# youdie006/CLAP2Diffusion

Measured on AMD Instinct MI355X. Metric: 512x512 images/sec @ 50 DDIM steps, batch=8, 1/2/4/8 MI355X, higher is better.
Workload: dtype fp16; 1 GPU; c3: batch=8/GPU, 50 DDIM steps, 512x512, CFG 7.5, log-mel+HTSAT+projectors+CLIP+UNet+VAE, all-gather of images; global_batch=8, ddim_steps=50, resolution=512, parallelism=dp1

## Files before the change

clap2diffusion_amd/_lib.py:

```python
from __future__ import annotations

import ctypes
import os
from ctypes import c_float, c_int, c_size_t, c_void_p
from pathlib import Path

import torch

LIB_PATH = Path(os.environ.get("C2D_LIB") or Path(__file__).resolve().parent / "libc2d_hip.so")

C2D_PRO_NONE, C2D_PRO_GN, C2D_PRO_LN, C2D_PRO_SILU, C2D_PRO_LNFOLD = 0, 1, 2, 3, 4
C2D_PAD_SAME, C2D_PAD_AFTER = 0, 1
C2D_ACT = {None: 0, "none": 0, "geglu": 1, "gelu": 2, "relu": 3, "silu": 4, "quick_gelu": 5}
ERRORS = {-1: "C2D_E_ARG", -2: "C2D_E_SHAPE", -3: "C2D_E_ALIGN", -4: "C2D_E_HIP"}

EXPORTS = [
    "c2d_conv2d_igemm", "c2d_conv2d_igemm_workspace_size", "c2d_conv2d_igemm_plan", "c2d_set_plan_override", "c2d_get_plan_override", "c2d_groupnorm_workspace_size", "c2d_groupnorm_stats", "c2d_groupnorm_apply", "c2d_groupnorm_run_workspace_size", "c2d_groupnorm", "c2d_groupnorm_pad_workspace_size", "c2d_groupnorm_pad", "c2d_conv2d_gn_rows", "c2d_groupnorm_moments", "c2d_layernorm_stats",
    "c2d_layernorm", "c2d_attention_fwd", "c2d_attention_fwd_bias", "c2d_attention_fwd_mask", "c2d_window_attention", "c2d_htsat_mel_patches",
    "c2d_patch_merge_gather", "c2d_row_mean", "c2d_l2_normalize", "c2d_softmax_rows", "c2d_clap_log_mel", "c2d_attention_small", "c2d_pack_weights", "c2d_timestep_embedding",
    "c2d_cfg_ddim_step", "c2d_latent_to_nhwc", "c2d_upsample_nearest2x", "c2d_add", "c2d_last_hip_error", "c2d_version",
    "c2d_image_to_nhwc", "c2d_vae_posterior_noise",
    "c2d_cfg_ddim_step_masked", "c2d_mask_to_latent", "c2d_composite_u8",
    "c2d_inpaint_prepare",
]


class ConvDesc(ctypes.Structure):
    _fields_ = [
        ("src0", c_void_p), ("src1", c_void_p), ("c0", c_int), ("c1", c_int),
        ("n", c_int), ("h", c_int), ("w", c_int), ("oh", c_int), ("ow", c_int),
        ("ksize", c_int), ("stride", c_int), ("up", c_int),
        ("weight", c_void_p), ("cout", c_int), ("kpad", c_int),
        ("pro", c_int), ("pro_silu", c_int), ("pro_a", c_void_p), ("pro_b", c_void_p),
        ("gamma", c_void_p), ("beta", c_void_p), ("bias", c_void_p), ("act", c_int),
        ("temb", c_void_p), ("temb_ld", c_int), ("resid", c_void_p), ("resid_ld", c_int),
        ("out", c_void_p), ("out_ld", c_int), ("ws", c_void_p), ("ws_bytes", c_size_t),
        ("src_pad", c_int), ("pro_eps", c_float),
        ("gn_mom", c_void_p), ("gn_groups", c_int),
        ("pad_mode", c_int),
    ]


_lib = None


def lib() -> ctypes.CDLL:
    global _lib
    if _lib is not None:
        return _lib
    if not LIB_PATH.exists():
        raise RuntimeError(
            f"{LIB_PATH} is missing: build it with `python -m clap2diffusion_amd.build` "
            "(the HIP library is the only compute path; there is no fallback)")
    L = ctypes.CDLL(str(LIB_PATH))
    vp, i, f, sz = c_void_p, c_int, c_float, c_size_t
    sig = {
        "c2d_conv2d_igemm": ([ctypes.POINTER(ConvDesc), vp], i),
        "c2d_conv2d_igemm_workspace_size": ([ctypes.POINTER(ConvDesc)], sz),
        "c2d_conv2d_igemm_plan": ([ctypes.POINTER(ConvDesc), ctypes.POINTER(c_int), ctypes.POINTER(c_int)], i),
        "c2d_set_plan_override": ([i, i], i),
        "c2d_get_plan_override": ([ctypes.POINTER(ctypes.c_int), ctypes.POINTER(ctypes.c_int)], i),
        "c2d_groupnorm_workspace_size": ([i, i, i], sz),
        "c2d_groupnorm_stats": ([vp, vp, i, i, i, i, i, f, vp, vp, vp, vp, vp, vp], i),
        "c2d_groupnorm_apply": ([vp, vp, i, i, i, i, vp, vp, i, vp, vp], i),
        "c2d_groupnorm_run_workspace_size": ([i, i, i, i], sz),
        "c2d_groupnorm": ([vp, vp, i, i, i, i, i, f, vp, vp, i, vp, vp, sz, vp], i),
        "c2d_groupnorm_pad_workspace_size": ([i, i, i, i], sz),
        "c2d_groupnorm_pad": ([vp, vp, i, i, i, i, i, i, f, vp, vp, i, vp, vp, sz, vp], i),
        "c2d_conv2d_gn_rows": ([ctypes.POINTER(ConvDesc)], i),
        "c2d_groupnorm_moments": ([vp, i, i, i, i, f, vp, vp, i, vp, i, i, vp, vp], i),
        "c2d_layernorm_stats": ([vp, i, i, i, f, vp, vp], i),
        "c2d_layernorm": ([vp, i, i, i, f, vp, vp, vp, i, vp], i),
        "c2d_attention_fwd": ([vp, i, vp, i, vp, i, vp, i, i, i, i, i, i, f, i, vp], i),
        "c2d_attention_fwd_bias": ([vp, i, vp, i, vp, i, vp, i, i, i, i, i, i, f, i, vp, i, i, vp], i),
        "c2d_attention_fwd_mask": ([vp, i, vp, i, vp, i, vp, i, i, i, i, i, i, f, i, vp, i, i, i, vp], i),
        "c2d_window_attention": ([vp, i, vp, i, i, i, vp, vp, i, vp, i, vp], i),
        "c2d_htsat_mel_patches": ([vp, i, i, vp, vp, vp, vp], i),
        "c2d_patch_merge_gather": ([vp, i, i, i, i, vp, vp], i),
        "c2d_row_mean": ([vp, i, i, i, i, vp, vp], i),
        "c2d_l2_normalize": ([vp, i, i, vp], i),
        "c2d_softmax_rows": ([vp, i, i, i, vp, i, vp], i),
        "c2d_clap_log_mel": ([vp, vp, vp, i, i, i, i, vp, vp, vp, i, vp, vp], i),
        "c2d_attention_small": ([vp, i, vp, i, vp, i, vp, i, i, i, i, i, f, i, vp], i),
        "c2d_pack_weights": ([vp, i, i, i, i, i, vp, vp], i),
        "c2d_timestep_embedding": ([vp, vp, i, i, vp, vp], i),
        "c2d_cfg_ddim_step": ([vp, vp, i, i, i, f, vp, vp, i, vp], i),
        "c2d_latent_to_nhwc": ([vp, i, i, i, i, i, vp, vp], i),
        "c2d_upsample_nearest2x": ([vp, i, i, i, i, vp, vp], i),
        "c2d_image_to_nhwc": ([vp, i, i, vp, vp], i),
        "c2d_vae_posterior_noise": ([vp, i, vp, vp, vp, vp, i, i, f, vp, vp], i),
        "c2d_cfg_ddim_step_masked": ([vp, vp, vp, vp, vp, i, i, i, f, vp, vp, i, vp], i),
        "c2d_mask_to_latent": ([vp, i, i, i, vp, vp], i),
        "c2d_composite_u8": ([vp, vp, vp, sz, vp, vp], i),
        "c2d_inpaint_prepare": ([vp, i, vp, vp, vp, vp, vp, i, i, i, i, f, vp, vp, vp, vp], i),
        "c2d_add": ([vp, vp, vp, sz, vp], i),
        "c2d_last_hip_error": ([], i),
        "c2d_version": ([], ctypes.c_char_p),
    }
    for name, (args, res) in sig.items():
        fn = getattr(L, name)
        fn.argtypes = args
        fn.restype = res
    _lib = L
    return L


def check(rc: int, what: str) -> None:
    if rc != 0:
        extra = ""
        if rc == -4:
            extra = f" (hipError {lib().c2d_last_hip_error()})"
        raise RuntimeError(f"{what} failed: {ERRORS.get(rc, rc)}{extra}")


def stream_ptr() -> int:
    return torch.cuda.current_stream().cuda_stream


def ptr(t) -> int | None:
    if t is None:
        return None
    return t.data_ptr()


def is_available() -> bool:
    return LIB_PATH.exists()


os.environ.setdefault("HSA_ENABLE_IPC_MODE_LEGACY", "0")
```

clap2diffusion_amd/csrc/norm.hip:

```cpp
#include "common.h"
#include <stdlib.h>

namespace c2d {

__device__ __forceinline__ float gn_read(const f16* s0, const f16* s1, int c0, int c1, size_t pix, int c) {
    return (float)((c < c0) ? s0[pix * c0 + c] : s1[pix * c1 + (c - c0)]);
}

template <int CPT, bool GP = false>
__global__ void __launch_bounds__(256) gn_partial_kernel(const f16* __restrict__ s0, const f16* __restrict__ s1,
                                                         int c0, int c1, int hw, int cpg, int rows_per_block,
                                                         float* __restrict__ ws) {
    extern __shared__ __attribute__((aligned(16))) float red[];
    const int cin = c0 + c1, nch = cin >> 3;
    const int n = blockIdx.y;
    const int t = threadIdx.x;
    const int R = (CPT == 1) ? (256 / nch) : 1;
    const int ch_base = (CPT == 1) ? (t % nch) : t;
    const int r0 = (CPT == 1) ? (t / nch) : 0;
    const bool active = (CPT == 1) ? (t < R * nch) : true;
    const int p_begin = blockIdx.x * rows_per_block;
    const int p_end = min(hw, p_begin + rows_per_block);
    const size_t img = (size_t)n * hw;

    float sum[CPT][8], sq[CPT][8], shift[CPT][8];
#pragma unroll
    for (int q = 0; q < CPT; ++q)
#pragma unroll
        for (int i = 0; i < 8; ++i) { sum[q][i] = 0.f; sq[q][i] = 0.f; shift[q][i] = 0.f; }

    if (active) {
        auto ld8 = [&](int pix, int q) {
            const size_t gp = img + pix;
            const int c = (ch_base + q * 256) * 8;
            const f16* ptr = (c < c0) ? (s0 + gp * c0 + c) : (s1 + gp * c1 + (c - c0));
            return *reinterpret_cast<const f16x8*>(ptr);
        };
        auto acc8 = [&](const f16x8& v, int q) {
#pragma unroll
            for (int i = 0; i < 8; ++i) {
                float d = (float)v[i] - shift[q][i];
                sum[q][i] += d;
                sq[q][i] += d * d;
            }
        };
        constexpr int UN = CPT == 1 ? 8 : 4;
        int pix = p_begin + r0;
        bool first = true;
        for (; pix + (UN - 1) * R < p_end; pix += UN * R) {
            f16x8 v[UN][CPT];
#pragma unroll
            for (int u = 0; u < UN; ++u)
#pragma unroll
                for (int q = 0; q < CPT; ++q)
                    if (q == 0 || ch_base + q * 256 < nch) v[u][q] = ld8(pix + u * R, q);
            if (first) {
#pragma unroll
                for (int q = 0; q < CPT; ++q) {
                    const int ch = ch_base + q * 256;
                    if (ch >= nch) continue;
#pragma unroll
                    for (int i = 0; i < 8; ++i) shift[q][i] = gn_read(s0, s1, c0, c1, img, ((ch * 8 + i) / cpg) * cpg);
                }
                first = false;
            }
            asm volatile("" ::: "memory");
#pragma unroll
            for (int u = 0; u < UN; ++u)
#pragma unroll
                for (int q = 0; q < CPT; ++q)
                    if (q == 0 || ch_base + q * 256 < nch) acc8(v[u][q], q);
        }
        if (first) {
#pragma unroll
            for (int q = 0; q < CPT; ++q) {
                const int ch = ch_base + q * 256;
                if (ch >= nch) continue;
#pragma unroll
                for (int i = 0; i < 8; ++i) shift[q][i] = gn_read(s0, s1, c0, c1, img, ((ch * 8 + i) / cpg) * cpg);
            }
        }
        for (; pix < p_end; pix += R) {
#pragma unroll
            for (int q = 0; q < CPT; ++q)
                if (q == 0 || ch_base + q * 256 < nch) acc8(ld8(pix, q), q);
        }
    }
    if constexpr (GP) {
        float* chs = red + (CPT == 1 ? R * cin * 2 : 0);
        if (CPT == 1) {
            if (active) {
#pragma unroll
                for (int i = 0; i < 8; ++i) {
                    red[(r0 * cin + ch_base * 8 + i) * 2 + 0] = sum[0][i];
                    red[(r0 * cin + ch_base * 8 + i) * 2 + 1] = sq[0][i];
                }
            }
            __syncthreads();
            for (int c = t; c < cin; c += 256) {
                float a = 0.f, b = 0.f;
                for (int r = 0; r < R; ++r) { a += red[(r * cin + c) * 2]; b += red[(r * cin + c) * 2 + 1]; }
                chs[c * 2] = a;
                chs[c * 2 + 1] = b;
            }
        } else {
#pragma unroll
            for (int q = 0; q < CPT; ++q) {
                const int ch = ch_base + q * 256;
                if (ch >= nch) continue;
#pragma unroll
                for (int i = 0; i < 8; ++i) { chs[(ch * 8 + i) * 2] = sum[q][i]; chs[(ch * 8 + i) * 2 + 1] = sq[q][i]; }
            }
        }
        __syncthreads();
        const int groups = cin / cpg;
        float* dst = ws + ((size_t)n * gridDim.x + blockIdx.x) * groups * 2;
        for (int g = t; g < groups; g += 256) {
            float a = 0.f, b = 0.f;
            for (int i = 0; i < cpg; ++i) { a += chs[(g * cpg + i) * 2]; b += chs[(g * cpg + i) * 2 + 1]; }
            dst[g * 2] = a;
            dst[g * 2 + 1] = b;
        }
        return;
    }
    if (CPT == 1) {
        if (active) {
#pragma unroll
            for (int i = 0; i < 8; ++i) {
                red[(r0 * cin + ch_base * 8 + i) * 2 + 0] = sum[0][i];
                red[(r0 * cin + ch_base * 8 + i) * 2 + 1] = sq[0][i];
            }
        }
        __syncthreads();
        float* dst = ws + (((size_t)n * gridDim.x + blockIdx.x) * cin) * 2;
        for (int c = t; c < cin; c += 256) {
            float a = 0.f, b = 0.f;
            for (int r = 0; r < R; ++r) { a += red[(r * cin + c) * 2]; b += red[(r * cin + c) * 2 + 1]; }
            dst[c * 2 + 0] = a;
            dst[c * 2 + 1] = b;
        }
    } else {
#pragma unroll
        for (int q = 0; q < CPT; ++q) {
            const int ch = ch_base + q * 256;
            if (ch >= nch) continue;
            float* dst = ws + (((size_t)n * gridDim.x + blockIdx.x) * cin + ch * 8) * 2;
#pragma unroll
            for (int i = 0; i < 8; ++i) { dst[i * 2] = sum[q][i]; dst[i * 2 + 1] = sq[q][i]; }
        }
    }
}

__host__ __device__ inline int gn_tpc(int cpg) { return cpg <= 64 ? 4 : (cpg <= 128 ? 2 : 1); }

__global__ void __launch_bounds__(256) gn_finalize_kernel(const f16* __restrict__ s0, const f16* __restrict__ s1,
                                                          int c0, int c1, int hw, int groups, int nblk, float eps,
                                                          const float* __restrict__ gamma, const float* __restrict__ beta,
                                                          const float* __restrict__ ws, float* __restrict__ scale,
                                                          float* __restrict__ shift) {
    __shared__ double csum[256], csq[256];
    __shared__ float g_mean[256], g_rstd[256];
    const int cin = c0 + c1, cpg = cin / groups;
    const int tpc = gn_tpc(cpg);
    const int gpb = 256 / (cpg * tpc);
    const int n = blockIdx.x, g0 = blockIdx.y * gpb;
    const int ng = min(gpb, groups - g0);
    const int c_begin = g0 * cpg, nc = ng * cpg;
    const int t = threadIdx.x;
    const int cs = t / tpc, part = t - cs * tpc;
    const size_t img = (size_t)n * hw;
    const float2* wp = reinterpret_cast<const float2*>(ws) + (size_t)n * nblk * cin + c_begin + (cs < nc ? cs : 0);
    double a = 0.0, b = 0.0;
    if (cs < nc) {
        int blk = part;
        for (; blk + 3 * tpc < nblk; blk += 4 * tpc) {
            const float2 v0 = wp[(size_t)blk * cin], v1 = wp[(size_t)(blk + tpc) * cin];
            const float2 v2 = wp[(size_t)(blk + 2 * tpc) * cin], v3 = wp[(size_t)(blk + 3 * tpc) * cin];
            a += (double)v0.x; b += (double)v0.y;
            a += (double)v1.x; b += (double)v1.y;
            a += (double)v2.x; b += (double)v2.y;
            a += (double)v3.x; b += (double)v3.y;
        }
        for (; blk < nblk; blk += tpc) {
            const float2 v = wp[(size_t)blk * cin];
            a += (double)v.x; b += (double)v.y;
        }
    }
    for (int o = 1; o < tpc; o <<= 1) {
        a += __shfl_xor(a, o);
        b += __shfl_xor(b, o);
    }
    if (cs < nc && part == 0) {
        csum[cs] = a;
        csq[cs] = b;
    }
    __syncthreads();
    if (t < ng) {
        double a = 0.0, b = 0.0;
        for (int i = 0; i < cpg; ++i) { a += csum[t * cpg + i]; b += csq[t * cpg + i]; }
        const double cnt = (double)hw * cpg;
        const double m1 = a / cnt;
        double var = b / cnt - m1 * m1;
        if (var < 0.0) var = 0.0;
        const float sft = gn_read(s0, s1, c0, c1, img, (g0 + t) * cpg);
        g_mean[t] = (float)(sft + m1);
        g_rstd[t] = (float)(1.0 / sqrt(var + (double)eps));
    }
    __syncthreads();
    if (t < nc) {
        const int c = c_begin + t, gl = t / cpg;
        const float sc = gamma[c] * g_rstd[gl];
        scale[(size_t)n * cin + c] = sc;
        shift[(size_t)n * cin + c] = beta[c] - g_mean[gl] * sc;
    }
}

template <int CPT, bool PAD = false>
__global__ void __launch_bounds__(256) gn_apply_kernel(const f16* __restrict__ s0, const f16* __restrict__ s1, int c0,
                                                       int c1, int hw, const float* __restrict__ scale,
                                                       const float* __restrict__ shift, int silu, f16* __restrict__ out,
                                                       int pw = 0) {
    const int cin = c0 + c1, nch = cin >> 3;
    const int L = nch < 256 ? nch : 256, R = 256 / L;
    const int t = threadIdx.x, lane_c = t % L, r0 = t / L;
    if (r0 >= R) return;
    const int n = blockIdx.y;
    const size_t img = (size_t)n * hw;
    float av[CPT][8], bv[CPT][8];
    const f16* src[CPT];
    int ld[CPT], cc[CPT];
    bool on[CPT];
#pragma unroll
    for (int q = 0; q < CPT; ++q) {
        const int ch = lane_c + q * 256;
        on[q] = ch < nch;
        cc[q] = (on[q] ? ch : 0) * 8;
        const int c = cc[q];
        src[q] = (c < c0) ? (s0 + c) : (s1 + (c - c0));
        ld[q] = (c < c0) ? c0 : c1;
#pragma unroll
        for (int i = 0; i < 8; ++i) {
            av[q][i] = scale[(size_t)n * cin + c + i];
            bv[q][i] = shift[(size_t)n * cin + c + i];
        }
    }
    if constexpr (PAD) {
        const int w = pw - 2, ph = hw / w + 2, npix = ph * pw;
        const size_t pimg = (size_t)n * npix;
#pragma unroll 2
        for (int pp = blockIdx.x * R + r0; pp < npix; pp += gridDim.x * R) {
            const int py = pp / pw, px = pp - py * pw;
            const bool inner = py >= 1 && py < ph - 1 && px >= 1 && px < pw - 1;
            const size_t gp = img + (inner ? (py - 1) * w + (px - 1) : 0);
#pragma unroll
            for (int q = 0; q < CPT; ++q) {
                if (!on[q]) continue;
                f16x8 o = (f16x8){0, 0, 0, 0, 0, 0, 0, 0};
                if (inner) {
                    const f16x8 v = *reinterpret_cast<const f16x8*>(src[q] + gp * ld[q]);
#pragma unroll
                    for (int j = 0; j < 8; ++j) {
                        float y = fmaf((float)v[j], av[q][j], bv[q][j]);
                        if (silu) y = y * __builtin_amdgcn_rcpf(1.0f + __expf(-y));
                        o[j] = (f16)y;
                    }
                }
                *reinterpret_cast<f16x8*>(out + (pimg + pp) * cin + cc[q]) = o;
            }
        }
        return;
    }
#pragma unroll 4
    for (int pix = blockIdx.x * R + r0; pix < hw; pix += gridDim.x * R) {
        const size_t gp = img + pix;
#pragma unroll
        for (int q = 0; q < CPT; ++q) {
            if (!on[q]) continue;
            const f16x8 v = *reinterpret_cast<const f16x8*>(src[q] + gp * ld[q]);
            f16x8 o;
#pragma unroll
            for (int j = 0; j < 8; ++j) {
                float y = fmaf((float)v[j], av[q][j], bv[q][j]);
                if (silu) y = y * __builtin_amdgcn_rcpf(1.0f + __expf(-y));
                o[j] = (f16)y;
            }
            *reinterpret_cast<f16x8*>(out + gp * cin + cc[q]) = o;
        }
    }
}

template <int CPT, bool PAD, bool MOM = false>
__global__ void __launch_bounds__(256) gn_apply_fold_kernel(const f16* __restrict__ s0, const f16* __restrict__ s1,
                                                            int c0, int c1, int hw, int cpg, int nblk, float eps,
                                                            const float* __restrict__ gamma,
                                                            const float* __restrict__ beta,
                                                            const float* __restrict__ ws, int silu,
                                                            f16* __restrict__ out, int pw = 0, int mrows = 0) {
    __shared__ double dacc[MOM ? 768 : 512];
    __shared__ float gmr[512];
    const int cin = c0 + c1, nch = cin >> 3, groups = cin / cpg;
    const int L = nch < 256 ? nch : 256, R = 256 / L;
    const int t = threadIdx.x, lane_c = t % L, r0 = t / L;
    const int n = blockIdx.y;
    const size_t img = (size_t)n * hw;
    const int parts = 256 / groups;
    if constexpr (MOM) {
        const double nb = (double)mrows * cpg;
        if (t < parts * groups) {
            const int g = t % groups, pt = t / groups;
            const float2* wp = reinterpret_cast<const float2*>(ws) + (size_t)n * nblk * groups + g;
            const double sh = (double)wp[0].x;
            double a = 0.0, b = 0.0, qq = 0.0;
            for (int k = pt; k < nblk; k += parts) {
                const float2 v = wp[(size_t)k * groups];
                const double d = (double)v.x - sh;
                a += d;
                b += d * d;
                qq += (double)v.y;
            }
            dacc[t * 3] = a;
            dacc[t * 3 + 1] = b;
            dacc[t * 3 + 2] = qq;
        }
        __syncthreads();
        if (t < groups) {
            double a = 0.0, b = 0.0, qq = 0.0;
            for (int pt = 0; pt < parts; ++pt) {
                const int u = (pt * groups + t) * 3;
                a += dacc[u];
                b += dacc[u + 1];
                qq += dacc[u + 2];
            }
            const float2* wp = reinterpret_cast<const float2*>(ws) + (size_t)n * nblk * groups + t;
            const double K = (double)nblk;
            double var = (qq + nb * (b - a * a / K)) / (K * nb);
            if (var < 0.0) var = 0.0;
            gmr[t * 2] = (float)((double)wp[0].x + a / K);
            gmr[t * 2 + 1] = (float)(1.0 / sqrt(var + (double)eps));
        }
    } else {
    if (t < parts * groups) {
        const int g = t % groups, pt = t / groups;
        const float2* wp = reinterpret_cast<const float2*>(ws) + (size_t)n * nblk * groups + g;
        double a = 0.0, b = 0.0;
        int k = pt;
        for (; k + 3 * parts < nblk; k += 4 * parts) {
            const float2 v0 = wp[(size_t)k * groups], v1 = wp[(size_t)(k + parts) * groups];
            const float2 v2 = wp[(size_t)(k + 2 * parts) * groups], v3 = wp[(size_t)(k + 3 * parts) * groups];
            a += (double)v0.x; b += (double)v0.y;
            a += (double)v1.x; b += (double)v1.y;
            a += (double)v2.x; b += (double)v2.y;
            a += (double)v3.x; b += (double)v3.y;
        }
        for (; k < nblk; k += parts) {
            const float2 v = wp[(size_t)k * groups];
            a += (double)v.x; b += (double)v.y;
        }
        dacc[t * 2] = a;
        dacc[t * 2 + 1] = b;
    }
    __syncthreads();
    if (t < groups) {
        double a = 0.0, b = 0.0;
        for (int pt = 0; pt < parts; ++pt) { a += dacc[(pt * groups + t) * 2]; b += dacc[(pt * groups + t) * 2 + 1]; }
        const double cnt = (double)hw * cpg;
        const double m1 = a / cnt;
        double var = b / cnt - m1 * m1;
        if (var < 0.0) var = 0.0;
        gmr[t * 2] = (float)(gn_read(s0, s1, c0, c1, img, t * cpg) + m1);
        gmr[t * 2 + 1] = (float)(1.0 / sqrt(var + (double)eps));
    }
    }
    __syncthreads();
    if (r0 >= R) return;
    float av[CPT][8], bv[CPT][8];
    const f16* src[CPT];
    int ld[CPT], cc[CPT];
    bool on[CPT];
#pragma unroll
    for (int q = 0; q < CPT; ++q) {
        const int ch = lane_c + q * 256;
        on[q] = ch < nch;
        cc[q] = (on[q] ? ch : 0) * 8;
        const int c = cc[q];
        src[q] = (c < c0) ? (s0 + c) : (s1 + (c - c0));
        ld[q] = (c < c0) ? c0 : c1;
#pragma unroll
        for (int i = 0; i < 8; ++i) {
            const int gl = (c + i) / cpg;
            const float sc = gamma[c + i] * gmr[gl * 2 + 1];
            av[q][i] = sc;
            bv[q][i] = beta[c + i] - gmr[gl * 2] * sc;
        }
    }
    if constexpr (PAD) {
        const int w = pw - 2, ph = hw / w + 2, npix = ph * pw;
        const size_t pimg = (size_t)n * npix;
#pragma unroll 2
        for (int pp = blockIdx.x * R + r0; pp < npix; pp += gridDim.x * R) {
            const int py = pp / pw, px = pp - py * pw;
            const bool inner = py >= 1 && py < ph - 1 && px >= 1 && px < pw - 1;
            const size_t gp = img + (inner ? (py - 1) * w + (px - 1) : 0);
#pragma unroll
            for (int q = 0; q < CPT; ++q) {
                if (!on[q]) continue;
                f16x8 o = (f16x8){0, 0, 0, 0, 0, 0, 0, 0};
                if (inner) {
                    const f16x8 v = *reinterpret_cast<const f16x8*>(src[q] + gp * ld[q]);
#pragma unroll
                    for (int j = 0; j < 8; ++j) {
                        float y = fmaf((float)v[j], av[q][j], bv[q][j]);
                        if (silu) y = y * __builtin_amdgcn_rcpf(1.0f + __expf(-y));
                        o[j] = (f16)y;
                    }
                }
                *reinterpret_cast<f16x8*>(out + (pimg + pp) * cin + cc[q]) = o;
            }
        }
        return;
    }
#pragma unroll 4
    for (int pix = blockIdx.x * R + r0; pix < hw; pix += gridDim.x * R) {
        const size_t gp = img + pix;
#pragma unroll
        for (int q = 0; q < CPT; ++q) {
            if (!on[q]) continue;
            const f16x8 v = *reinterpret_cast<const f16x8*>(src[q] + gp * ld[q]);
            f16x8 o;
#pragma unroll
            for (int j = 0; j < 8; ++j) {
                float y = fmaf((float)v[j], av[q][j], bv[q][j]);
                if (silu) y = y * __builtin_amdgcn_rcpf(1.0f + __expf(-y));
                o[j] = (f16)y;
            }
            *reinterpret_cast<f16x8*>(out + gp * cin + cc[q]) = o;
        }
    }
}

template <int NT>
__global__ void __launch_bounds__(NT) gn_fused_kernel(const f16* __restrict__ s0, const f16* __restrict__ s1, int c0,
                                                      int c1, int hw, int cpg, int cb, float eps,
                                                      const float* __restrict__ gamma, const float* __restrict__ beta,
                                                      int silu, f16* __restrict__ out) {
    __shared__ float red[2 * 2048];
    __shared__ double gsum[256], gsq[256];
    __shared__ float aff[2 * 256];
    const int cin = c0 + c1;
    const int L = cb >> 3, R = NT / L, R1 = 256 / L;
    const int n = blockIdx.y, cbase = blockIdx.x * cb;
    const int t = threadIdx.x, lane_c = t % L, r0 = t / L;
    const bool active = r0 < R && cbase + lane_c * 8 < cin;
    const int c = cbase + lane_c * 8;
    const size_t img = (size_t)n * hw;
    const f16* src = (c < c0) ? (s0 + c) : (s1 + (c - c0));
    const int ld = (c < c0) ? c0 : c1;
    float sh[8], sum[8], sq[8];
#pragma unroll
    for (int i = 0; i < 8; ++i) { sum[i] = 0.f; sq[i] = 0.f; sh[i] = 0.f; }
    if (active) {
#pragma unroll
        for (int i = 0; i < 8; ++i) sh[i] = gn_read(s0, s1, c0, c1, img, ((c + i) / cpg) * cpg);
#pragma unroll 4
        for (int pix = r0; pix < hw; pix += R) {
            const f16x8 v = *reinterpret_cast<const f16x8*>(src + (img + pix) * ld);
#pragma unroll
            for (int i = 0; i < 8; ++i) {
                const float d = (float)v[i] - sh[i];
                sum[i] += d;
                sq[i] += d * d;
            }
        }
    }
    const int nph = (R + R1 - 1) / R1;
    for (int ph = 0; ph < nph; ++ph) {
        if (r0 < R && r0 / R1 == ph) {
            float* dst = red + ((r0 - ph * R1) * cb + lane_c * 8) * 2;
#pragma unroll
            for (int i = 0; i < 8; ++i) {
                if (ph == 0) {
                    dst[i * 2] = sum[i];
                    dst[i * 2 + 1] = sq[i];
                } else {
                    dst[i * 2] += sum[i];
                    dst[i * 2 + 1] += sq[i];
                }
            }
        }
        __syncthreads();
    }
    const int rs = R < R1 ? R : R1;
    if (t < cb) {
        double a = 0.0, b = 0.0;
        for (int r = 0; r < rs; ++r) { a += (double)red[(r * cb + t) * 2]; b += (double)red[(r * cb + t) * 2 + 1]; }
        gsum[t] = a;
        gsq[t] = b;
    }
    __syncthreads();
    if (t < cb && cbase + t < cin) {
        const int gl = t / cpg;
        double a = 0.0, b = 0.0;
        for (int i = 0; i < cpg; ++i) { a += gsum[gl * cpg + i]; b += gsq[gl * cpg + i]; }
        const double cnt = (double)hw * cpg;
        const double m1 = a / cnt;
        double var = b / cnt - m1 * m1;
        if (var < 0.0) var = 0.0;
        const float mean = (float)(gn_read(s0, s1, c0, c1, img, cbase + gl * cpg) + m1);
        const float rstd = (float)(1.0 / sqrt(var + (double)eps));
        const float scl = gamma[cbase + t] * rstd;
        aff[t] = scl;
        aff[256 + t] = beta[cbase + t] - mean * scl;
    }
    __syncthreads();
    if (!active) return;
    float av[8], bv[8];
#pragma unroll
    for (int i = 0; i < 8; ++i) { av[i] = aff[lane_c * 8 + i]; bv[i] = aff[256 + lane_c * 8 + i]; }
#pragma unroll 4
    for (int pix = r0; pix < hw; pix += R) {
        const f16x8 v = *reinterpret_cast<const f16x8*>(src + (img + pix) * ld);
        f16x8 o;
#pragma unroll
        for (int i = 0; i < 8; ++i) {
            float y = fmaf((float)v[i], av[i], bv[i]);
            if (silu) y = y * __builtin_amdgcn_rcpf(1.0f + __expf(-y));
            o[i] = (f16)y;
        }
        *reinterpret_cast<f16x8*>(out + (img + pix) * cin + c) = o;
    }
}

template <int NCH, bool APPLY>
__global__ void __launch_bounds__(256) ln_kernel(const f16* __restrict__ x, int m, int c, int ld, float eps,
                                                 float* __restrict__ stats, const float* __restrict__ gamma,
                                                 const float* __restrict__ beta, f16* __restrict__ out, int out_ld) {
    const int lane = threadIdx.x & 63;
    const int row = blockIdx.x * 4 + (threadIdx.x >> 6);
    if (row >= m) return;
    const int nch = c >> 3;
    const f16* xr = x + (size_t)row * ld;
    f16x8 v[NCH];
    float s = 0.f;
#pragma unroll
    for (int q = 0; q < NCH; ++q) {
        const int ch = lane + q * 64;
        if (ch < nch) {
            v[q] = *reinterpret_cast<const f16x8*>(xr + ch * 8);
#pragma unroll
            for (int i = 0; i < 8; ++i) s += (float)v[q][i];
        }
    }
    const float mean = wave_sum(s) / (float)c;
    float s2 = 0.f;
#pragma unroll
    for (int q = 0; q < NCH; ++q) {
        const int ch = lane + q * 64;
        if (ch < nch) {
#pragma unroll
            for (int i = 0; i < 8; ++i) { float d = (float)v[q][i] - mean; s2 += d * d; }
        }
    }
    const float rstd = rsqrtf(wave_sum(s2) / (float)c + eps);
    if (!APPLY) {
        if (lane == 0) { stats[(size_t)row * 2] = mean; stats[(size_t)row * 2 + 1] = rstd; }
        return;
    }
#pragma unroll
    for (int q = 0; q < NCH; ++q) {
        const int ch = lane + q * 64;
        if (ch < nch) {
            f16x8 o;
#pragma unroll
            for (int i = 0; i < 8; ++i) {
                const int cc = ch * 8 + i;
                o[i] = (f16)(((float)v[q][i] - mean) * rstd * gamma[cc] + beta[cc]);
            }
            *reinterpret_cast<f16x8*>(out + (size_t)row * out_ld + ch * 8) = o;
        }
    }
}

template <int LPR, int CPL>
__global__ void __launch_bounds__(256) ln_rows_kernel(const f16* __restrict__ x, int m, int ld, float eps,
                                                      const float* __restrict__ gamma, const float* __restrict__ beta,
                                                      f16* __restrict__ out, int out_ld) {
    constexpr int C = 8 * LPR * CPL;
    constexpr int RPW = 64 / LPR;
    const int lane = threadIdx.x & 63;
    const int sub = lane % LPR, rw = lane / LPR;
    const int wave_g = blockIdx.x * 4 + (threadIdx.x >> 6);
    const int nwaves = gridDim.x * 4;
    float g[CPL][8], b[CPL][8];
#pragma unroll
    for (int k = 0; k < CPL; ++k) {
        const int c = (sub + k * LPR) * 8;
#pragma unroll
        for (int i = 0; i < 8; i += 4) {
            const float4 gg = *reinterpret_cast<const float4*>(gamma + c + i);
            const float4 bb = *reinterpret_cast<const float4*>(beta + c + i);
            g[k][i] = gg.x; g[k][i + 1] = gg.y; g[k][i + 2] = gg.z; g[k][i + 3] = gg.w;
            b[k][i] = bb.x; b[k][i + 1] = bb.y; b[k][i + 2] = bb.z; b[k][i + 3] = bb.w;
        }
    }
    for (int row0 = wave_g * RPW; row0 < m; row0 += nwaves * RPW) {
        const int row = row0 + rw;
        const bool ok = row < m;
        const f16* xr = x + (size_t)(ok ? row : 0) * ld;
        f16x8 v[CPL];
        float s = 0.f;
#pragma unroll
        for (int k = 0; k < CPL; ++k) {
            v[k] = *reinterpret_cast<const f16x8*>(xr + (sub + k * LPR) * 8);
#pragma unroll
            for (int i = 0; i < 8; ++i) s += (float)v[k][i];
        }
#pragma unroll
        for (int o = 1; o < LPR; o <<= 1) s += __shfl_xor(s, o);
        const float mean = s * (1.0f / C);
        float s2 = 0.f;
#pragma unroll
        for (int k = 0; k < CPL; ++k)
#pragma unroll
            for (int i = 0; i < 8; ++i) { const float d = (float)v[k][i] - mean; s2 += d * d; }
#pragma unroll
        for (int o = 1; o < LPR; o <<= 1) s2 += __shfl_xor(s2, o);
        const float rstd = rsqrtf(s2 * (1.0f / C) + eps);
        if (!ok) continue;
#pragma unroll
        for (int k = 0; k < CPL; ++k) {
            f16x8 o;
#pragma unroll
            for (int i = 0; i < 8; ++i) o[i] = (f16)(((float)v[k][i] - mean) * rstd * g[k][i] + b[k][i]);
            *reinterpret_cast<f16x8*>(out + (size_t)row * out_ld + (sub + k * LPR) * 8) = o;
        }
    }
}

static int ln_rows_launch(const void* x, int m, int c, int ld, float eps, const float* gamma, const float* beta,
                          void* out, int out_ld, hipStream_t s) {
    if ((ld & 7) || (out_ld & 7) || !aligned16(gamma) || !aligned16(beta)) return 1;
    const int nch = c >> 3;
    int cpl = 0, lpr = 0;
    for (int cp : {5, 3}) {
        if (nch % cp) continue;
        const int l = nch / cp;
        if (l == 4 || l == 8 || l == 16 || l == 32) { cpl = cp; lpr = l; break; }
    }
    if (!cpl) return 1;
    const int rows_per_block = 4 * (64 / lpr);
    long want = ((long)m + rows_per_block - 1) / rows_per_block;
    const unsigned blocks = (unsigned)(want < 4096 ? want : 4096);
#define C2D_LNR(L, P)                                                                                            \
    if (lpr == L && cpl == P) {                                                                                  \
        hipLaunchKernelGGL((ln_rows_kernel<L, P>), dim3(blocks), dim3(256), 0, s, (const f16*)x, m, ld, eps, gamma, \
                           beta, (f16*)out, out_ld);                                                             \
        return check_launch();                                                                                   \
    }
    C2D_LNR(4, 3) C2D_LNR(8, 3) C2D_LNR(16, 3) C2D_LNR(32, 3)
    C2D_LNR(4, 5) C2D_LNR(8, 5) C2D_LNR(16, 5) C2D_LNR(32, 5)
#undef C2D_LNR
    return 1;
}

template <bool APPLY>
static int ln_dispatch(const void* x, int m, int c, int ld, float eps, float* stats, const float* gamma,
                       const float* beta, void* out, int out_ld, hipStream_t s) {
    if (APPLY) {
        const int rc = ln_rows_launch(x, m, c, ld, eps, gamma, beta, out, out_ld, s);
        if (rc != 1) return rc;
    }
    const int nch = c >> 3;
    dim3 grid((m + 3) / 4);
    if (nch <= 64)
        hipLaunchKernelGGL((ln_kernel<1, APPLY>), grid, dim3(256), 0, s, (const f16*)x, m, c, ld, eps, stats, gamma, beta, (f16*)out, out_ld);
    else if (nch <= 128)
        hipLaunchKernelGGL((ln_kernel<2, APPLY>), grid, dim3(256), 0, s, (const f16*)x, m, c, ld, eps, stats, gamma, beta, (f16*)out, out_ld);
    else if (nch <= 256)
        hipLaunchKernelGGL((ln_kernel<4, APPLY>), grid, dim3(256), 0, s, (const f16*)x, m, c, ld, eps, stats, gamma, beta, (f16*)out, out_ld);
    else if (nch <= 512)
        hipLaunchKernelGGL((ln_kernel<8, APPLY>), grid, dim3(256), 0, s, (const f16*)x, m, c, ld, eps, stats, gamma, beta, (f16*)out, out_ld);
    else
        return C2D_E_SHAPE;
    return check_launch();
}

}

using namespace c2d;

static int gn_target_blocks() { return tuning().gn_blocks; }

static int gn_apply_blocks() { return tuning().gn_apply_blocks; }

static int gn_rows_per_block(int n, int c, int hw, int cap = 32) {
    const int nch = c >> 3;
    const int r = nch <= 256 ? 256 / nch : 1;
    const long tb = gn_target_blocks();
    long want = ((long)n * hw + tb - 1) / tb;
    if (want < (hw + cap - 1) / cap) want = (hw + cap - 1) / cap;
    if (want < r) want = r;
    if (want > 128) want = 128;
    return (int)((want + r - 1) / r * r);
}

static int gn_blocks(int n, int c, int hw, int cap = 32) {
    const int rpb = gn_rows_per_block(n, c, hw, cap);
    return (hw + rpb - 1) / rpb;
}

extern "C" size_t c2d_groupnorm_workspace_size(int n, int c, int hw) {
    if (n <= 0 || c <= 0 || hw <= 0) return 0;
    return (size_t)n * gn_blocks(n, c, hw) * c * 2 * sizeof(float);
}

extern "C" int c2d_groupnorm_stats(const void* src0, const void* src1, int c0, int c1, int n, int hw, int groups,
                                   float eps, const float* gamma, const float* beta, float* scale, float* shift,
                                   void* ws, void* stream) {
    if (!src0 || !gamma || !beta || !scale || !shift || !ws) return C2D_E_ARG;
    if (c1 > 0 && !src1) return C2D_E_ARG;
    const int cin = c0 + c1;
    if ((c0 & 7) || (c1 & 7) || cin <= 0 || groups <= 0 || cin % groups) return C2D_E_SHAPE;
    if (cin / groups > 256 || n <= 0 || hw <= 0) return C2D_E_SHAPE;
    if (!aligned16(src0) || (src1 && !aligned16(src1))) return C2D_E_ALIGN;
    hipStream_t s = (hipStream_t)stream;
    const int nch = cin >> 3;
    const int cpg = cin / groups;
    const int rows_per_block = gn_rows_per_block(n, cin, hw);
    const int nblk = gn_blocks(n, cin, hw);
    dim3 grid(nblk, n);
    if (nch <= 256) {
        const int R = 256 / nch;
        const size_t lds = (size_t)R * cin * 2 * sizeof(float);
        hipLaunchKernelGGL((gn_partial_kernel<1>), grid, dim3(256), lds, s, (const f16*)src0, (const f16*)src1, c0, c1,
                           hw, cpg, rows_per_block, (float*)ws);
    } else {
        hipLaunchKernelGGL((gn_partial_kernel<2>), grid, dim3(256), 0, s, (const f16*)src0, (const f16*)src1, c0, c1,
                           hw, cpg, rows_per_block, (float*)ws);
    }
    const int gpb = 256 / (cpg * gn_tpc(cpg));
    hipLaunchKernelGGL(gn_finalize_kernel, dim3(n, (groups + gpb - 1) / gpb), dim3(256), 0, s, (const f16*)src0, (const f16*)src1, c0, c1, hw,
                       groups, nblk, eps, gamma, beta, (const float*)ws, scale, shift);
    return check_launch();
}

extern "C" int c2d_layernorm_stats(const void* x, int m, int c, int ld, float eps, float* stats, void* stream) {
    if (!x || !stats) return C2D_E_ARG;
    if ((c & 7) || (ld & 7) || c <= 0) return C2D_E_SHAPE;
    if (!aligned16(x)) return C2D_E_ALIGN;
    if (m <= 0) return C2D_OK;
    return ln_dispatch<false>(x, m, c, ld, eps, stats, nullptr, nullptr, nullptr, 0, (hipStream_t)stream);
}

extern "C" int c2d_layernorm(const void* x, int m, int c, int ld, float eps, const float* gamma, const float* beta,
                             void* out, int out_ld, void* stream) {
    if (!x || !gamma || !beta || !out) return C2D_E_ARG;
    if ((c & 7) || (ld & 7) || (out_ld & 7) || c <= 0) return C2D_E_SHAPE;
    if (!aligned16(x) || !aligned16(out)) return C2D_E_ALIGN;
    if (m <= 0) return C2D_OK;
    return ln_dispatch<true>(x, m, c, ld, eps, nullptr, gamma, beta, out, out_ld, (hipStream_t)stream);
}

extern "C" int c2d_groupnorm_apply(const void* src0, const void* src1, int c0, int c1, int n, int hw,
                                   const float* scale, const float* shift, int silu, void* out, void* stream) {
    if (!src0 || !scale || !shift || !out) return C2D_E_ARG;
    if (c1 > 0 && !src1) return C2D_E_ARG;
    if ((c0 & 7) || (c1 & 7) || c0 + c1 <= 0 || n <= 0 || hw <= 0) return C2D_E_SHAPE;
    if (!aligned16(src0) || (src1 && !aligned16(src1)) || !aligned16(out) || !aligned16(scale) || !aligned16(shift))
        return C2D_E_ALIGN;
    const int nch = (c0 + c1) >> 3;
    if (nch > 512) return C2D_E_SHAPE;
    const int L = nch < 256 ? nch : 256, R = 256 / L;
    int bx = (gn_apply_blocks() + n - 1) / n;
    const int maxb = (hw + R - 1) / R;
    if (bx > maxb) bx = maxb;
    if (bx < 1) bx = 1;
    if (nch <= 256)
        hipLaunchKernelGGL(gn_apply_kernel<1>, dim3(bx, n), dim3(256), 0, (hipStream_t)stream, (const f16*)src0,
                           (const f16*)src1, c0, c1, hw, scale, shift, silu, (f16*)out);
    else
        hipLaunchKernelGGL(gn_apply_kernel<2>, dim3(bx, n), dim3(256), 0, (hipStream_t)stream, (const f16*)src0,
                           (const f16*)src1, c0, c1, hw, scale, shift, silu, (f16*)out);
    return check_launch();
}

static int gn_fused_cb(int n, int cin, int groups) {
    const int cpg = cin / groups;
    int u = cpg;
    while (u % 8) u += cpg;
    if (u > 256) return 0;
    int cb = u;
    while (cb * 2 <= 256 && cin % (cb * 2) == 0 && (long)n * (cin / (cb * 2)) >= 256) cb *= 2;
    return cb;
}

static int gn_fused_max_hw() { return tuning().gn_fused_hw; }

static bool gn_use_fused(int n, int cin, int hw, int groups) {
    return gn_fused_cb(n, cin, groups) > 0 && hw <= gn_fused_max_hw();
}


static bool gn_use_fold(int n, int cin, int hw, int groups) {
    (void)n; (void)hw;
    return tuning().gn_fold != 0 && groups <= 256 && (cin >> 3) <= 512;
}

static int gn_fold_run(const void* src0, const void* src1, int c0, int c1, int n, int hw, int pw, int groups,
                       float eps, const float* gamma, const float* beta, int silu, void* out, void* ws, hipStream_t s) {
    const int cin = c0 + c1, nch = cin >> 3, cpg = cin / groups;
    const int cap = tuning().gn_fold_cap;
    const int rows_per_block = gn_rows_per_block(n, cin, hw, cap);
    const int nblk = gn_blocks(n, cin, hw, cap);
    const dim3 pgrid(nblk, n);
    if (nch <= 256) {
        const size_t lds = ((size_t)(256 / nch) * cin * 2 + (size_t)cin * 2) * sizeof(float);
        hipLaunchKernelGGL((gn_partial_kernel<1, true>), pgrid, dim3(256), lds, s, (const f16*)src0, (const f16*)src1,
                           c0, c1, hw, cpg, rows_per_block, (float*)ws);
    } else {
        hipLaunchKernelGGL((gn_partial_kernel<2, true>), pgrid, dim3(256), (size_t)cin * 2 * sizeof(float), s,
                           (const f16*)src0, (const f16*)src1, c0, c1, hw, cpg, rows_per_block, (float*)ws);
    }
    const int L = nch < 256 ? nch : 256, R = 256 / L;
    const int npix = pw ? (hw / (pw - 2) + 2) * pw : hw;
    int bx = ((n < 8 ? tuning().gn_fold_apply_blocks : gn_apply_blocks()) + n - 1) / n;
    const int maxb = (npix + R - 1) / R;
    if (bx > maxb) bx = maxb;
    if (bx < 1) bx = 1;
    const dim3 agrid(bx, n);
#define C2D_GNF(C, PD)                                                                                           \
    hipLaunchKernelGGL((gn_apply_fold_kernel<C, PD>), agrid, dim3(256), 0, s, (const f16*)src0, (const f16*)src1, c0, \
                       c1, hw, cpg, nblk, eps, gamma, beta, (const float*)ws, silu, (f16*)out, pw)
    if (nch <= 256) {
        if (pw) C2D_GNF(1, true); else C2D_GNF(1, false);
    } else {
        if (pw) C2D_GNF(2, true); else C2D_GNF(2, false);
    }
#undef C2D_GNF
    return check_launch();
}

extern "C" int c2d_groupnorm_moments(const void* src, int c, int n, int hw, int groups, float eps, const float* gamma,
                                     const float* beta, int silu, const float* mom, int rows, int pw, void* out,
                                     void* stream) {
    if (!src || !gamma || !beta || !mom || !out) return C2D_E_ARG;
    if ((c & 7) || c <= 0 || (c >> 3) > 512 || groups <= 0 || groups > 256 || c % groups || n <= 0 || hw <= 0)
        return C2D_E_SHAPE;
    if (rows <= 0 || hw % rows) return C2D_E_SHAPE;
    if (pw && (pw < 3 || hw % (pw - 2))) return C2D_E_SHAPE;
    if (!aligned16(src) || !aligned16(out) || ((uintptr_t)mom & 7)) return C2D_E_ALIGN;
    const int nch = c >> 3, cpg = c / groups, nblk = hw / rows;
    const int L = nch < 256 ? nch : 256, R = 256 / L;
    const int npix = pw ? (hw / (pw - 2) + 2) * pw : hw;
    int bx = ((n < 8 ? tuning().gn_fold_apply_blocks : gn_apply_blocks()) + n - 1) / n;
    const int maxb = (npix + R - 1) / R;
    if (bx > maxb) bx = maxb;
    if (bx < 1) bx = 1;
    const dim3 agrid(bx, n);
    hipStream_t s = (hipStream_t)stream;
#define C2D_GNM(C, PD)                                                                                            \
    hipLaunchKernelGGL((gn_apply_fold_kernel<C, PD, true>), agrid, dim3(256), 0, s, (const f16*)src, (const f16*)nullptr, \
                       c, 0, hw, cpg, nblk, eps, gamma, beta, mom, silu, (f16*)out, pw, rows)
    if (nch <= 256) {
        if (pw) C2D_GNM(1, true); else C2D_GNM(1, false);
    } else {
        if (pw) C2D_GNM(2, true); else C2D_GNM(2, false);
    }
#undef C2D_GNM
    return check_launch();
}

static size_t gn_fold_ws_bytes(int n, int c, int hw, int groups) {
    return (size_t)n * gn_blocks(n, c, hw, tuning().gn_fold_cap) * groups * 2 * sizeof(float);
}

extern "C" size_t c2d_groupnorm_run_workspace_size(int n, int c, int hw, int groups) {
    if (n <= 0 || c <= 0 || hw <= 0 || groups <= 0 || c % groups) return 0;
    if (gn_use_fused(n, c, hw, groups)) return 0;
    const size_t multi = c2d_groupnorm_workspace_size(n, c, hw) + (size_t)n * c * 2 * sizeof(float);
    const size_t fold = gn_fold_ws_bytes(n, c, hw, groups);
    return fold > multi ? fold : multi;
}

extern "C" int c2d_groupnorm(const void* src0, const void* src1, int c0, int c1, int n, int hw, int groups, float eps,
                             const float* gamma, const float* beta, int silu, void* out, void* ws, size_t ws_bytes,
                             void* stream) {
    if (!src0 || !gamma || !beta || !out) return C2D_E_ARG;
    if (c1 > 0 && !src1) return C2D_E_ARG;
    const int cin = c0 + c1;
    if ((c0 & 7) || (c1 & 7) || cin <= 0 || groups <= 0 || cin % groups) return C2D_E_SHAPE;
    if (cin / groups > 256 || n <= 0 || hw <= 0) return C2D_E_SHAPE;
    if (!aligned16(src0) || (src1 && !aligned16(src1)) || !aligned16(out)) return C2D_E_ALIGN;
    hipStream_t s = (hipStream_t)stream;
    if (gn_use_fused(n, cin, hw, groups)) {
        const int cb = gn_fused_cb(n, cin, groups);
        hipLaunchKernelGGL(gn_fused_kernel<256>, dim3((cin + cb - 1) / cb, n), dim3(256), 0, s, (const f16*)src0,
                           (const f16*)src1, c0, c1, hw, cin / groups, cb, eps, gamma, beta, silu, (f16*)out);
        return check_launch();
    }
    if (!ws || ws_bytes < c2d_groupnorm_run_workspace_size(n, cin, hw, groups) || !aligned16(ws)) return C2D_E_ARG;
    if (gn_use_fold(n, cin, hw, groups))
        return gn_fold_run(src0, src1, c0, c1, n, hw, 0, groups, eps, gamma, beta, silu, out, ws, s);
    const size_t part = c2d_groupnorm_workspace_size(n, cin, hw);
    float* scale = reinterpret_cast<float*>(static_cast<char*>(ws) + part);
    float* shift = scale + (size_t)n * cin;
    int rc = c2d_groupnorm_stats(src0, src1, c0, c1, n, hw, groups, eps, gamma, beta, scale, shift, ws, stream);
    if (rc != C2D_OK) return rc;
    return c2d_groupnorm_apply(src0, src1, c0, c1, n, hw, scale, shift, silu, out, stream);
}

extern "C" size_t c2d_groupnorm_pad_workspace_size(int n, int c, int h, int w) {
    if (n <= 0 || c <= 0 || h <= 0 || w <= 0) return 0;
    const size_t multi = c2d_groupnorm_workspace_size(n, c, h * w) + (size_t)n * c * 2 * sizeof(float);
    const size_t fold = gn_fold_ws_bytes(n, c, h * w, c < 256 ? c : 256);
    return fold > multi ? fold : multi;
}

extern "C" int c2d_groupnorm_pad(const void* src0, const void* src1, int c0, int c1, int n, int h, int w, int groups,
                                 float eps, const float* gamma, const float* beta, int silu, void* out, void* ws,
                                 size_t ws_bytes, void* stream) {
    if (!src0 || !gamma || !beta || !out || !ws) return C2D_E_ARG;
    if (c1 > 0 && !src1) return C2D_E_ARG;
    const int cin = c0 + c1;
    if ((c0 & 7) || (c1 & 7) || cin <= 0 || groups <= 0 || cin % groups) return C2D_E_SHAPE;
    if (cin / groups > 256 || n <= 0 || h <= 0 || w <= 0 || (cin >> 3) > 512) return C2D_E_SHAPE;
    if (!aligned16(src0) || (src1 && !aligned16(src1)) || !aligned16(out) || !aligned16(ws)) return C2D_E_ALIGN;
    const int hw = h * w;
    if (ws_bytes < c2d_groupnorm_pad_workspace_size(n, cin, h, w)) return C2D_E_ARG;
    if (gn_use_fold(n, cin, hw, groups))
        return gn_fold_run(src0, src1, c0, c1, n, hw, w + 2, groups, eps, gamma, beta, silu, out, ws,
                           (hipStream_t)stream);
    const size_t part = c2d_groupnorm_workspace_size(n, cin, hw);
    float* scale = reinterpret_cast<float*>(static_cast<char*>(ws) + part);
    float* shift = scale + (size_t)n * cin;
    int rc = c2d_groupnorm_stats(src0, src1, c0, c1, n, hw, groups, eps, gamma, beta, scale, shift, ws, stream);
    if (rc != C2D_OK) return rc;
    const int nch = cin >> 3;
    const int L = nch < 256 ? nch : 256, R = 256 / L;
    const int npix = (h + 2) * (w + 2);
    int bx = (gn_apply_blocks() + n - 1) / n;
    const int maxb = (npix + R - 1) / R;
    if (bx > maxb) bx = maxb;
    if (bx < 1) bx = 1;
    if (nch <= 256)
        hipLaunchKernelGGL((gn_apply_kernel<1, true>), dim3(bx, n), dim3(256), 0, (hipStream_t)stream, (const f16*)src0,
                           (const f16*)src1, c0, c1, hw, scale, shift, silu, (f16*)out, w + 2);
    else
        hipLaunchKernelGGL((gn_apply_kernel<2, true>), dim3(bx, n), dim3(256), 0, (hipStream_t)stream, (const f16*)src0,
                           (const f16*)src1, c0, c1, hw, scale, shift, silu, (f16*)out, w + 2);
    return check_launch();
}
```

clap2diffusion_amd/layers.py:

```python
from __future__ import annotations

import torch
import torch.nn as nn

from . import ops


class HLinear(nn.Module):
    def __init__(self, in_features: int, out_features: int, bias: bool = True):
        super().__init__()
        self.in_features, self.out_features = in_features, out_features
        self.kpad = ops.kpad_of(in_features)
        self.register_buffer("weight", torch.zeros(out_features, self.kpad, dtype=torch.float16))
        self.register_buffer("bias", torch.zeros(out_features, dtype=torch.float32) if bias else None)

    @torch.no_grad()
    def load(self, w: torch.Tensor, b: torch.Tensor | None = None) -> None:
        wp, kp = ops.pack_linear_weight(w.float())
        assert kp == self.kpad and wp.shape[0] == self.out_features
        self.weight.copy_(wp)
        if self.bias is not None:
            self.bias.copy_(b.float() if b is not None else torch.zeros_like(self.bias))

    def forward(self, x: torch.Tensor, **kw) -> torch.Tensor:
        shp = x.shape
        x2 = x.reshape(-1, shp[-1])
        if not x2.is_contiguous():
            x2 = x2.contiguous()
        out = ops.conv(x2, self.weight, self.kpad, self.out_features, ksize=1, bias=self.bias, **kw)
        return out.view(*shp[:-1], out.shape[-1])


class HConv2d(nn.Module):

    def __init__(self, cin: int, cout: int, ksize: int, stride: int = 1, cin_pad: int | None = None,
                 pad_after: bool = False):
        super().__init__()
        assert not pad_after or (ksize == 3 and stride == 2)
        self.cin, self.cout, self.ksize, self.stride, self.pad_after = cin, cout, ksize, stride, pad_after
        self.cin_pad = cin_pad or cin
        self.kpad = ops.kpad_of(ksize * ksize * self.cin_pad)
        self.register_buffer("weight", torch.zeros(cout, self.kpad, dtype=torch.float16))
        self.register_buffer("bias", torch.zeros(cout, dtype=torch.float32))

    @torch.no_grad()
    def load(self, w: torch.Tensor, b: torch.Tensor | None) -> None:
        wp, kp = ops.pack_conv_weight(w.float(), cin_pad=self.cin_pad if self.cin_pad != self.cin else None)
        assert kp == self.kpad, (kp, self.kpad)
        self.weight.copy_(wp)
        if b is not None:
            self.bias.copy_(b.float())

    def forward(self, x: torch.Tensor, **kw) -> torch.Tensor:
        if self.pad_after:
            kw["pad_after"] = True
        return ops.conv(x, self.weight, self.kpad, self.cout, ksize=self.ksize, stride=self.stride, bias=self.bias, **kw)


class HUpConv2d(HConv2d):

    def __init__(self, cin: int, cout: int):
        super().__init__(cin, cout, 3)
        self.kpad_fold = 4 * cin
        self.register_buffer("weight_fold", torch.zeros(4, cout, self.kpad_fold, dtype=torch.float16), persistent=False)

    @torch.no_grad()
    def load(self, w: torch.Tensor, b: torch.Tensor | None) -> None:
        super().load(w, b)
        wf, kp = ops.fold_upsample_weight(w.float())
        assert kp == self.kpad_fold
        self.weight_fold.copy_(wf)

    def forward_folded(self, x: torch.Tensor) -> torch.Tensor:
        return ops.conv(x, self.weight_fold, self.kpad_fold, self.cout, ksize=3, bias=self.bias, up_fold=True)


class HGroupNorm(nn.Module):

    def __init__(self, num_groups: int, num_channels: int, eps: float):
        super().__init__()
        self.num_groups, self.num_channels, self.eps = num_groups, num_channels, eps
        self.register_buffer("weight", torch.ones(num_channels))
        self.register_buffer("bias", torch.zeros(num_channels))

    @torch.no_grad()
    def load(self, w, b):
        self.weight.copy_(w.float())
        self.bias.copy_(b.float())

    def stats(self, x: torch.Tensor, x2: torch.Tensor | None = None):
        return ops.group_norm_stats(x, self.num_groups, self.eps, self.weight, self.bias, x2=x2)

    def apply(self, x: torch.Tensor, x2: torch.Tensor | None = None, silu: bool = False,
              pad: bool = False, mom=None) -> torch.Tensor:
        return ops.group_norm(x, self.num_groups, self.eps, self.weight, self.bias, silu, x2=x2, pad=pad, mom=mom)


class HLayerNorm(nn.Module):
    def __init__(self, c: int, eps: float = 1e-5):
        super().__init__()
        self.c, self.eps = c, eps
        self.register_buffer("weight", torch.ones(c))
        self.register_buffer("bias", torch.zeros(c))

    @torch.no_grad()
    def load(self, w, b):
        self.weight.copy_(w.float())
        self.bias.copy_(b.float())

    def forward(self, x: torch.Tensor) -> torch.Tensor:
        shp = x.shape
        return ops.layer_norm(x.reshape(-1, shp[-1]), self.weight, self.bias, self.eps).view(shp)

    def prologue(self, x2d: torch.Tensor):
        return ops.layer_norm_stats(x2d, self.eps), self.weight, self.bias


def load_tree(module: nn.Module, sd: dict, prefix: str = "") -> list[str]:
    used = []
    for name, m in module.named_modules():
        if isinstance(m, (HLinear, HConv2d, HGroupNorm, HLayerNorm)):
            key = (prefix + name) if name else prefix.rstrip(".")
            wk, bk = key + ".weight", key + ".bias"
            if wk not in sd:
                raise KeyError(f"missing weight {wk}")
            m.load(sd[wk], sd.get(bk))
            used.append(wk)
            if bk in sd:
                used.append(bk)
    return used
```

clap2diffusion_amd/ops.py:

```python
from __future__ import annotations

import ctypes
import functools
import math

import torch

from . import torch_ops
from ._lib import C2D_ACT

C2D = torch.ops.c2d

F16 = torch.float16


def _require(t: torch.Tensor, name: str) -> None:
    if not t.is_cuda:
        raise RuntimeError(f"{name} must be a device tensor (HIP path only, no CPU fallback)")


def kpad_of(k: int) -> int:
    return (k + 63) // 64 * 64


def pack_conv_weight(w: torch.Tensor, cin_pad: int | None = None) -> tuple[torch.Tensor, int]:
    cout, cin, kh, kw = w.shape
    if cin_pad and cin_pad > cin:
        w = torch.nn.functional.pad(w, (0, 0, 0, 0, 0, cin_pad - cin))
        cin = cin_pad
    k = kh * kw * cin
    wp = w.permute(0, 2, 3, 1).reshape(cout, k)
    kp = kpad_of(k)
    if kp > k:
        wp = torch.nn.functional.pad(wp, (0, kp - k))
    return wp.to(F16).contiguous(), kp


def pack_weights_device(w: torch.Tensor, cin_pad: int | None = None) -> tuple[torch.Tensor, int]:
    _require(w, "w")
    w = w.float().contiguous()
    cout, cin = w.shape[:2]
    ks = w.shape[2] if w.dim() == 4 else 1
    cp = max(cin_pad or cin, cin)
    kp = kpad_of(ks * ks * cp)
    out = torch.empty(cout, kp, device=w.device, dtype=F16)
    C2D.pack_weights(w, cout, cin, ks, cp, kp, out)
    return out, kp


def pack_linear_weight(w: torch.Tensor) -> tuple[torch.Tensor, int]:
    out_f, in_f = w.shape
    kp = kpad_of(in_f)
    wp = torch.nn.functional.pad(w, (0, kp - in_f)) if kp > in_f else w
    return wp.to(F16).contiguous(), kp


_UPFOLD_TAPS = (((0,), (1, 2)), ((0, 1), (2,)))


@torch.no_grad()
def fold_upsample_weight(w: torch.Tensor, dtype: torch.dtype = F16) -> tuple[torch.Tensor, int]:
    cout, cin, kh, kw = w.shape
    assert kh == 3 and kw == 3
    out = w.new_zeros(4, cout, 2, 2, cin)
    for a in range(2):
        for b in range(2):
            for ty in range(2):
                for tx in range(2):
                    acc = out[2 * a + b, :, ty, tx, :]
                    for ky in _UPFOLD_TAPS[a][ty]:
                        for kx in _UPFOLD_TAPS[b][tx]:
                            acc += w[:, :, ky, kx]
    return out.reshape(4, cout, 4 * cin).to(dtype).contiguous(), 4 * cin


@functools.lru_cache(maxsize=None)
def upfold_ok(n: int, h: int, w: int, cin: int, cout: int) -> bool:
    import ctypes
    from ._lib import ConvDesc, lib
    d = ConvDesc()
    d.c0, d.n, d.h, d.w, d.oh, d.ow, d.ksize, d.stride, d.up = cin, n, h, w, 2 * h, 2 * w, 3, 1, 2
    d.cout, d.kpad, d.out_ld = cout, 4 * cin, cout
    tid, ks = ctypes.c_int(), ctypes.c_int()
    return lib().c2d_conv2d_igemm_plan(ctypes.byref(d), ctypes.byref(tid), ctypes.byref(ks)) == 0


def geglu_interleave(w: torch.Tensor, b: torch.Tensor | None):
    two_i = w.shape[0]
    inner = two_i // 2
    assert inner % 16 == 0
    idx = torch.arange(two_i).view(2, inner // 16, 16).permute(1, 0, 2).reshape(-1)
    wi = w[idx]
    bi = b[idx] if b is not None else None
    return wi, bi


def conv(x: torch.Tensor, weight: torch.Tensor, kpad: int, cout: int, *, ksize: int, bias=None, stride: int = 1,
         up: bool = False, x2: torch.Tensor | None = None, gn=None, gn_silu: bool = False, ln=None,
         silu_in: bool = False, act: str | None = None, temb: torch.Tensor | None = None,
         resid: torch.Tensor | None = None, out: torch.Tensor | None = None, padded: bool = False,
         ln_fold=None, gn_moments: int = 0, up_fold: bool = False, pad_after: bool = False):
    _require(x, "x")
    if x.dim() == 2:
        h, w = 1, x.shape[0]
    else:
        _, h, w, _ = x.shape
        if padded:
            assert ksize == 3 and stride == 1 and not up and x2 is None, "padded source: 3x3, stride 1, one source"
            assert gn is None and ln is None and not silu_in, "padded source: no GN / LN / SiLU prologue"
            h, w = h - 2, w - 2
    assert x.is_contiguous() and x.dtype == F16
    if x2 is not None:
        assert x2.is_contiguous() and x2.dtype == F16 and x2.shape[:-1] == x.shape[:-1]
    if up_fold:
        assert ksize == 3 and stride == 1 and not up and not padded and x2 is None and x.dim() == 4
        assert gn is None and ln is None and not silu_in and act is None and temb is None and resid is None
        assert not gn_moments and not ln_fold
    if pad_after:
        assert ksize == 3 and stride == 2 and not up and not up_fold and not padded and x.dim() == 4
        assert h % 2 == 0 and w % 2 == 0, "pad-after downsample: even H and W"
    if ksize == 3:
        vh, vw = (2 * h, 2 * w) if up or up_fold else (h, w)
        oh, ow = (vh + 2 - 3) // stride + 1, (vw + 2 - 3) // stride + 1
    else:
        oh, ow = h, w
    out_cols = cout // 2 if act == "geglu" else cout
    if out is None:
        shape = (x.shape[0], out_cols) if x.dim() == 2 else (x.shape[0], oh, ow, out_cols)
        out = torch.empty(shape, device=x.device, dtype=F16)
    assert out.stride(-1) == 1
    if resid is not None:
        assert resid.stride(-1) == 1
    gs, gh = gn if gn is not None else (None, None)
    ls, lg, lb = ln if ln is not None else (None, None, None)
    mom, rows = None, 0
    if gn_moments and x.dim() == 4 and act is None and not up and not pad_after and out.is_contiguous():
        rows = gn_moment_rows(out.shape[0], oh, ow, x.shape[-1], cout, ksize, stride, bool(padded), resid is not None,
                              temb is not None, gn_moments, x2.shape[-1] if x2 is not None else 0)
        if rows:
            mom = torch.empty((out.shape[0], oh * ow // rows, gn_moments, 2), device=x.device, dtype=torch.float32)
    C2D.conv2d_igemm(x, weight, kpad, cout, ksize, stride, up, x2, gs, gh, gn_silu, ls, lg, lb, silu_in, bias,
                     C2D_ACT[act], temb, resid, out, bool(padded), float(ln_fold or 0.0), mom, int(gn_moments),
                     bool(up_fold), bool(pad_after))
    if gn_moments:
        return out, (GnMoments(out, mom, rows, gn_moments) if mom is not None else None)
    return out


class GnMoments:

    def __init__(self, of: torch.Tensor, mom: torch.Tensor, rows: int, groups: int):
        self.of, self.mom, self.rows, self.groups = of, mom, rows, groups

    def matches(self, x: torch.Tensor, groups: int) -> bool:
        return (x is self.of and groups == self.groups and x.dim() == 4 and
                tuple(self.mom.shape[:1]) == tuple(x.shape[:1]))


@functools.lru_cache(maxsize=None)
def gn_moment_rows(n: int, oh: int, ow: int, cin: int, cout: int, ksize: int, stride: int, padded: bool, resid: bool,
                   temb: bool, groups: int, c1: int = 0) -> int:
    import ctypes
    from ._lib import ConvDesc, lib
    d = ConvDesc()
    h, w = (oh, ow) if padded or ksize == 1 or stride == 1 else (oh * stride, ow * stride)
    d.c0, d.n, d.h, d.w, d.oh, d.ow, d.ksize, d.stride, d.src_pad = cin, n, h, w, oh, ow, ksize, stride, int(padded)
    d.c1 = c1
    if c1:
        d.src1 = 256
    d.cout, d.kpad, d.out_ld = cout, kpad_of(ksize * ksize * (cin + c1)), cout
    d.out = 256
    if resid:
        d.resid, d.resid_ld = 256, cout
    if temb:
        d.temb, d.temb_ld = 256, cout
    d.ws, d.ws_bytes = 256, 1 << 40
    d.gn_groups = groups
    return int(lib().c2d_conv2d_gn_rows(ctypes.byref(d)))


@torch.no_grad()
def fold_layernorm(weight: torch.Tensor, bias: torch.Tensor | None, gamma: torch.Tensor, beta: torch.Tensor,
                   in_features: int):
    w = weight[:, :in_features].float()
    wp = torch.zeros_like(weight)
    wp[:, :in_features] = (w * gamma.float().view(1, -1)).to(F16)
    b = w @ beta.float()
    if bias is not None:
        b = b + bias.float()
    return wp.contiguous(), b.contiguous()


@functools.lru_cache(maxsize=None)
def panel_gemm(m: int, k: int, cout: int, geglu: bool, lnfold: bool = False) -> bool:
    import ctypes
    from ._lib import C2D_PRO_LNFOLD, ConvDesc, lib
    d = ConvDesc()
    d.c0, d.n, d.h, d.w, d.oh, d.ow, d.ksize, d.stride = k, 1, 1, m, 1, m, 1, 1
    d.cout, d.kpad, d.act = cout, kpad_of(k), C2D_ACT["geglu" if geglu else None]
    d.out_ld = cout // 2 if geglu else cout
    if lnfold:
        d.pro, d.pro_eps = C2D_PRO_LNFOLD, 1e-5
    tid, ks = ctypes.c_int(), ctypes.c_int()
    rc = lib().c2d_conv2d_igemm_plan(ctypes.byref(d), ctypes.byref(tid), ctypes.byref(ks))
    return rc == 0 and tid.value == 70


ROWRING_TILES = (42, 43, 44)


@functools.lru_cache(maxsize=None)
def rowring_conv(n: int, h: int, w: int, cin: int, cout: int) -> bool:
    import ctypes
    from ._lib import ConvDesc, check, lib
    d = ConvDesc()
    d.c0, d.n, d.h, d.w, d.oh, d.ow, d.ksize, d.stride = cin, n, h, w, h, w, 3, 1
    d.cout, d.kpad, d.src_pad = cout, kpad_of(9 * cin), 1
    d.out_ld = cout
    tid, ks = ctypes.c_int(), ctypes.c_int()
    check(lib().c2d_conv2d_igemm_plan(ctypes.byref(d), ctypes.byref(tid), ctypes.byref(ks)), "c2d_conv2d_igemm_plan")
    return tid.value in ROWRING_TILES


def conv_workspace_bytes(n: int, h: int, w: int, c0: int, c1: int, cout: int, ksize: int) -> int:
    import ctypes
    from ._lib import ConvDesc, lib
    d = ConvDesc()
    d.c0, d.c1, d.n, d.h, d.w, d.oh, d.ow, d.ksize, d.stride = c0, c1, n, h, w, h, w, ksize, 1
    d.cout, d.kpad, d.out_ld = cout, kpad_of(ksize * ksize * (c0 + c1)), cout
    return int(lib().c2d_conv2d_igemm_workspace_size(ctypes.byref(d)))


class record_conv_plans:

    def __enter__(self):
        self.plans = []
        torch_ops._plan_probe = self.plans
        return self.plans

    def __exit__(self, *exc):
        torch_ops._plan_probe = None
        return False


class force_plan:

    def __init__(self, tile: int, split: int = 0):
        self.tile, self.split = int(tile), int(split)

    def __enter__(self):
        import ctypes
        from ._lib import check, lib
        t, sp = ctypes.c_int(0), ctypes.c_int(0)
        check(lib().c2d_get_plan_override(ctypes.byref(t), ctypes.byref(sp)), "c2d_get_plan_override")
        self.prev = (t.value, sp.value)
        check(lib().c2d_set_plan_override(self.tile, self.split), "c2d_set_plan_override")
        rowring_conv.cache_clear()
        gn_moment_rows.cache_clear()
        return self

    def __exit__(self, *exc):
        from ._lib import lib
        lib().c2d_set_plan_override(*self.prev)
        rowring_conv.cache_clear()
        gn_moment_rows.cache_clear()
        return False


def plan_override_from_env() -> None:
    import os
    from ._lib import check, lib
    t, sp = int(os.environ.get("C2D_GEMM_TILE", "0") or 0), int(os.environ.get("C2D_GEMM_SPLIT", "0") or 0)
    if t or sp:
        check(lib().c2d_set_plan_override(t, sp), "c2d_set_plan_override")


def group_norm_stats(x: torch.Tensor, groups: int, eps: float, gamma: torch.Tensor, beta: torch.Tensor,
                     x2: torch.Tensor | None = None):
    _require(x, "x")
    c = x.shape[-1] + (x2.shape[-1] if x2 is not None else 0)
    scale = torch.empty((x.shape[0], c), device=x.device, dtype=torch.float32)
    shift = torch.empty_like(scale)
    C2D.groupnorm_stats(x, x2, groups, float(eps), gamma, beta, scale, shift)
    return scale, shift


def group_norm_apply(x: torch.Tensor, gn, silu: bool, x2: torch.Tensor | None = None,
                     out: torch.Tensor | None = None) -> torch.Tensor:
    _require(x, "x")
    c = x.shape[-1] + (x2.shape[-1] if x2 is not None else 0)
    if out is None:
        out = torch.empty((*x.shape[:-1], c), device=x.device, dtype=F16)
    C2D.groupnorm_apply(x, x2, gn[0], gn[1], bool(silu), out)
    return out


def group_norm(x: torch.Tensor, groups: int, eps: float, gamma: torch.Tensor, beta: torch.Tensor, silu: bool,
               x2: torch.Tensor | None = None, out: torch.Tensor | None = None, pad: bool = False,
               mom: "GnMoments | None" = None) -> torch.Tensor:
    _require(x, "x")
    c = x.shape[-1] + (x2.shape[-1] if x2 is not None else 0)
    if mom is not None and x2 is None and mom.matches(x, groups):
        n, h, w, _ = x.shape
        if out is None:
            out = torch.empty((n, h + 2, w + 2, c) if pad else x.shape, device=x.device, dtype=F16)
        C2D.groupnorm_moments(x, groups, float(eps), gamma, beta, bool(silu), mom.mom, mom.rows, bool(pad), out)
        return out
    if pad:
        n, h, w, _ = x.shape
        if out is None:
            out = torch.empty((n, h + 2, w + 2, c), device=x.device, dtype=F16)
        C2D.groupnorm_pad(x, x2, groups, float(eps), gamma, beta, bool(silu), out)
        return out
    if out is None:
        out = torch.empty((*x.shape[:-1], c), device=x.device, dtype=F16)
    C2D.groupnorm(x, x2, groups, float(eps), gamma, beta, bool(silu), out)
    return out


def layer_norm_stats(x2d: torch.Tensor, eps: float) -> torch.Tensor:
    _require(x2d, "x")
    st = torch.empty((x2d.shape[0], 2), device=x2d.device, dtype=torch.float32)
    C2D.layernorm_stats(x2d, float(eps), st)
    return st


def layer_norm(x2d: torch.Tensor, gamma: torch.Tensor, beta: torch.Tensor, eps: float,
               out: torch.Tensor | None = None) -> torch.Tensor:
    _require(x2d, "x")
    if out is None:
        out = torch.empty(x2d.shape, device=x2d.device, dtype=F16)
    C2D.layernorm(x2d, gamma, beta, float(eps), out)
    return out


def attention(q: torch.Tensor, k: torch.Tensor, v: torch.Tensor, batch: int, heads: int, lq: int, lk: int,
              d: int, scale: float | None = None, out: torch.Tensor | None = None,
              key_bias: torch.Tensor | None = None) -> torch.Tensor:
    _require(q, "q")
    if scale is None:
        scale = 1.0 / math.sqrt(d)
    if out is None:
        out = torch.empty((batch * lq, heads * d), device=q.device, dtype=F16)
    ldb = ldh = ldq = 0
    kb = None
    if key_bias is not None:
        kb = key_bias.to(device=q.device, dtype=torch.float32)
        if kb.dim() == 3:
            kb = kb.unsqueeze(2)
        if (kb.dim() != 4 or kb.shape[-1] != lk or kb.shape[0] not in (1, batch) or kb.shape[1] not in (1, heads)
                or kb.shape[2] not in (1, lq)):
            raise ValueError(f"key_bias must be [batch|1, heads|1, ({lq}|1,) {lk}], got {tuple(key_bias.shape)}")
        kb = kb.contiguous()
        ldb = kb.stride(0) if kb.shape[0] > 1 else 0
        ldh = kb.stride(1) if kb.shape[1] > 1 else 0
        ldq = kb.stride(2) if kb.shape[2] > 1 else 0
    C2D.attention_fwd(q, k, v, batch, heads, lq, lk, d, float(scale), kb, ldb, ldh, out, ldq)
    return out


def attention_small(q: torch.Tensor, k: torch.Tensor, v: torch.Tensor, batch: int, heads: int, l: int, d: int,
                    causal: bool, scale: float | None = None, out: torch.Tensor | None = None) -> torch.Tensor:
    _require(q, "q")
    if scale is None:
        scale = 1.0 / math.sqrt(d)
    if out is None:
        out = torch.empty((batch * l, heads * d), device=q.device, dtype=F16)
    C2D.attention_small(q, k, v, batch, heads, l, d, float(scale), bool(causal), out)
    return out


def window_attention(qkv: torch.Tensor, row_map: torch.Tensor, n_windows: int, heads: int, d: int,
                     bias: torch.Tensor, mask: torch.Tensor | None, out: torch.Tensor) -> torch.Tensor:
    C2D.window_attention(qkv, row_map, n_windows, heads, d, bias, mask, out)
    return out


def htsat_mel_patches(mel: torch.Tensor, bn_scale: torch.Tensor, bn_shift: torch.Tensor) -> torch.Tensor:
    b, t, f = mel.shape
    assert f == 64 and mel.dtype == torch.float32 and mel.is_contiguous()
    out = torch.empty((b * 4096, 64), device=mel.device, dtype=F16)
    C2D.htsat_mel_patches(mel, bn_scale, bn_shift, out)
    return out


def patch_merge_gather(x: torch.Tensor, b: int, h: int, w: int, c: int) -> torch.Tensor:
    out = torch.empty((b * (h // 2) * (w // 2), 4 * c), device=x.device, dtype=F16)
    C2D.patch_merge_gather(x, b, h, w, c, out)
    return out


def row_mean(x: torch.Tensor, b: int, rows: int) -> torch.Tensor:
    out = torch.empty((b, x.shape[1]), device=x.device, dtype=torch.float32)
    C2D.row_mean(x, b, rows, out)
    return out


def softmax_rows(x: torch.Tensor, out: torch.Tensor | None = None) -> torch.Tensor:
    _require(x, "x")
    assert x.dim() == 2 and x.dtype == F16 and x.stride(1) == 1
    out = torch.empty_like(x) if out is None else out
    assert out.shape == x.shape and out.stride(1) == 1
    C2D.softmax_rows(x, out)
    return out


def l2_normalize_(x: torch.Tensor) -> torch.Tensor:
    C2D.l2_normalize(x)
    return x


def timestep_embedding(t_table: torch.Tensor, step_index: torch.Tensor | None, n: int, dim: int) -> torch.Tensor:
    out = torch.empty((n, dim), device=t_table.device, dtype=F16)
    C2D.timestep_embedding(t_table, step_index, n, dim, out)
    return out


def cfg_ddim_step(eps: torch.Tensor, x: torch.Tensor, guidance: float, coef: torch.Tensor, step_index: torch.Tensor,
                  advance: bool = True) -> torch.Tensor:
    C2D.cfg_ddim_step(eps, x, float(guidance), coef, step_index, bool(advance))
    return x


def latent_to_nhwc(x: torch.Tensor, cpad: int, dup: bool) -> torch.Tensor:
    b, c, hgt, wid = x.shape
    out = torch.empty(((2 if dup else 1) * b, hgt, wid, cpad), device=x.device, dtype=F16)
    C2D.latent_to_nhwc(x, cpad, bool(dup), out)
    return out


def image_to_nhwc(img: torch.Tensor, out: torch.Tensor | None = None) -> torch.Tensor:
    _require(img, "img")
    assert img.dtype == torch.uint8 and img.dim() == 4 and img.shape[-1] == 3 and img.is_contiguous()
    if out is None:
        out = torch.empty((*img.shape[:-1], 8), device=img.device, dtype=F16)
    C2D.image_to_nhwc(img, out)
    return out


def vae_posterior_noise(moments: torch.Tensor, out: torch.Tensor, scaling: float, eps: torch.Tensor | None = None,
                        noise: torch.Tensor | None = None, coef: torch.Tensor | None = None,
                        step_index: torch.Tensor | None = None) -> torch.Tensor:
    _require(moments, "moments")
    assert moments.dim() == 2 and moments.dtype == F16 and moments.stride(1) == 1 and moments.shape[1] >= 8
    assert out.dtype == torch.float32 and out.is_contiguous() and out.dim() == 4 and out.shape[1] == 4
    assert moments.shape[0] == out.shape[0] * out.shape[2] * out.shape[3]
    for t in (eps, noise):
        assert t is None or (t.dtype == torch.float32 and t.is_contiguous() and t.shape == out.shape and t.is_cuda)
    if noise is not None:
        assert coef is not None and step_index is not None and coef.dtype == torch.float32
        assert step_index.dtype == torch.int32
    C2D.vae_posterior_noise(moments, eps, noise, coef, step_index, float(scaling), out)
    return out


def cfg_ddim_step_masked(eps: torch.Tensor, x: torch.Tensor, z0: torch.Tensor, noise: torch.Tensor, mask: torch.Tensor,
                         guidance: float, coef: torch.Tensor, step_index: torch.Tensor,
                         advance: bool = True) -> torch.Tensor:
    _require(x, "x")
    assert eps.dtype == F16 and eps.is_contiguous() and eps.numel() == 2 * x.numel()
    assert x.dim() == 4 and x.shape[1] == 4
    for t in (x, z0, noise):
        assert t.dtype == torch.float32 and t.is_contiguous() and t.shape == x.shape and t.is_cuda
    assert mask.dtype == torch.float32 and mask.is_contiguous() and mask.is_cuda
    assert tuple(mask.shape) == (x.shape[0], x.shape[2], x.shape[3])
    assert coef.dtype == torch.float32 and coef.is_contiguous() and coef.dim() == 2 and coef.shape[1] == 2
    assert step_index.dtype == torch.int32
    C2D.cfg_ddim_step_masked(eps, x, z0, noise, mask, float(guidance), coef, step_index, bool(advance))
    return x


def mask_to_latent(mask_u8: torch.Tensor, out: torch.Tensor | None = None) -> torch.Tensor:
    _require(mask_u8, "mask_u8")
    assert mask_u8.dtype == torch.uint8 and mask_u8.dim() == 3 and mask_u8.is_contiguous()
    n, hgt, wid = mask_u8.shape
    assert hgt % 8 == 0 and wid % 8 == 0 and hgt > 0 and wid > 0, f"mask size {hgt}x{wid} is no multiple of 8"
    if out is None:
        out = torch.empty((n, hgt // 8, wid // 8), device=mask_u8.device, dtype=torch.float32)
    assert out.dtype == torch.float32 and out.is_contiguous() and tuple(out.shape) == (n, hgt // 8, wid // 8)
    C2D.mask_to_latent(mask_u8, out)
    return out


def composite_u8(decoded: torch.Tensor, original: torch.Tensor, mask_u8: torch.Tensor,
                 out: torch.Tensor | None = None) -> torch.Tensor:
    _require(decoded, "decoded")
    for t in (decoded, original):
        assert t.dtype == torch.uint8 and t.is_contiguous() and t.is_cuda and t.shape == decoded.shape
    assert decoded.dim() == 4 and decoded.shape[-1] == 3
    assert mask_u8.dtype == torch.uint8 and mask_u8.is_contiguous() and mask_u8.is_cuda
    assert mask_u8.shape == decoded.shape[:-1]
    if out is None:
        out = torch.empty_like(decoded)
    assert out.dtype == torch.uint8 and out.is_contiguous() and out.shape == decoded.shape
    C2D.composite_u8(decoded, original, mask_u8, out)
    return out


def inpaint_prepare(moments: torch.Tensor, noise: torch.Tensor, mask_u8: torch.Tensor, scaling: float,
                    eps: torch.Tensor | None = None, coef: torch.Tensor | None = None,
                    step_index: torch.Tensor | None = None, pure_noise: bool = False, z0: torch.Tensor | None = None,
                    x: torch.Tensor | None = None, mask: torch.Tensor | None = None):
    _require(moments, "moments")
    assert moments.dim() == 2 and moments.dtype == F16 and moments.stride(1) == 1 and moments.shape[1] >= 8
    assert noise.dtype == torch.float32 and noise.is_contiguous() and noise.dim() == 4 and noise.shape[1] == 4
    n, _, hgt, wid = noise.shape
    assert moments.shape[0] == n * hgt * wid
    assert mask_u8.dtype == torch.uint8 and mask_u8.is_contiguous() and mask_u8.is_cuda
    assert tuple(mask_u8.shape) == (n, 8 * hgt, 8 * wid), f"mask {tuple(mask_u8.shape)} for latents {tuple(noise.shape)}"
    if z0 is None:
        z0 = torch.empty_like(noise)
    if x is None:
        x = torch.empty_like(noise)
    if mask is None:
        mask = torch.empty((n, hgt, wid), device=noise.device, dtype=torch.float32)
    for t in (eps, noise, z0, x):
        assert t is None or (t.dtype == torch.float32 and t.is_contiguous() and t.shape == noise.shape and t.is_cuda)
    assert x is not noise and x is not z0
    assert mask.dtype == torch.float32 and mask.is_contiguous() and tuple(mask.shape) == (n, hgt, wid)
    if not pure_noise:
        assert coef is not None and step_index is not None and coef.dtype == torch.float32
        assert step_index.dtype == torch.int32
    C2D.inpaint_prepare(moments, eps, noise, mask_u8, coef, step_index, bool(pure_noise), float(scaling), z0, x, mask)
    return z0, x, mask


def upsample_nearest2x(x: torch.Tensor, out: torch.Tensor | None = None) -> torch.Tensor:
    n, h, w, c = x.shape
    x = x.contiguous()
    if out is None:
        out = torch.empty(n, 2 * h, 2 * w, c, device=x.device, dtype=x.dtype)
    C2D.upsample_nearest2x(x, out)
    return out


def add(a: torch.Tensor, b: torch.Tensor, out: torch.Tensor | None = None) -> torch.Tensor:
    if out is None:
        out = torch.empty_like(a)
    C2D.add(a, b, out)
    return out
```

clap2diffusion_amd/torch_ops.py:

```python
import ctypes
from typing import Optional

import torch
from torch import Tensor
from torch.library import custom_op

from ._lib import C2D_PAD_AFTER, C2D_PAD_SAME, C2D_PRO_GN, C2D_PRO_LN, C2D_PRO_LNFOLD, C2D_PRO_NONE, C2D_PRO_SILU, ConvDesc, check, lib, ptr, stream_ptr

_CU = "cuda"


def _conv_desc(x, weight, kpad, cout, ksize, stride, up, x2, gn_scale, gn_shift, gn_silu, ln_stats, ln_gamma,
               ln_beta, silu_in, bias, act, temb, resid, out, src_pad=False, lnf_eps=0.0, gn_mom=None,
               gn_groups=0, up_fold=False, pad_after=False) -> ConvDesc:
    if x.dim() == 2:
        n, h, w = 1, 1, x.shape[0]
        c0 = x.shape[1]
    else:
        n, h, w, c0 = x.shape
        if src_pad:
            h, w = h - 2, w - 2
    c1 = x2.shape[-1] if x2 is not None else 0
    if ksize == 3:
        vh, vw = (2 * h, 2 * w) if up or up_fold else (h, w)
        oh, ow = (vh + 2 - 3) // stride + 1, (vw + 2 - 3) // stride + 1
        if pad_after:
            oh, ow = (h - 2) // 2 + 1, (w - 2) // 2 + 1
    else:
        oh, ow = h, w
    d = ConvDesc()
    d.src0 = ptr(x); d.src1 = ptr(x2); d.c0 = c0; d.c1 = c1
    d.n, d.h, d.w, d.oh, d.ow = n, h, w, oh, ow
    d.ksize, d.stride, d.up = ksize, stride, (2 if up_fold else int(up))
    d.weight = ptr(weight); d.cout = cout; d.kpad = kpad
    if lnf_eps > 0.0:
        d.pro = C2D_PRO_LNFOLD; d.pro_eps = lnf_eps
    elif gn_scale is not None:
        d.pro = C2D_PRO_GN; d.pro_silu = int(gn_silu); d.pro_a = ptr(gn_scale); d.pro_b = ptr(gn_shift)
    elif ln_stats is not None:
        d.pro = C2D_PRO_LN; d.pro_a = ptr(ln_stats); d.gamma = ptr(ln_gamma); d.beta = ptr(ln_beta)
    elif silu_in:
        d.pro = C2D_PRO_SILU
    else:
        d.pro = C2D_PRO_NONE
    d.bias = ptr(bias)
    d.act = act
    if temb is not None:
        d.temb = ptr(temb); d.temb_ld = temb.stride(0)
    if resid is not None:
        d.resid = ptr(resid); d.resid_ld = resid.stride(-2) if resid.dim() == 2 else resid.shape[-1]
    d.out = ptr(out)
    d.out_ld = out.stride(-2) if out.dim() == 2 else out.shape[-1]
    d.src_pad = int(src_pad)
    if gn_mom is not None:
        d.gn_mom = ptr(gn_mom); d.gn_groups = gn_groups
    d.pad_mode = C2D_PAD_AFTER if pad_after else C2D_PAD_SAME
    return d


_plan_probe: Optional[list] = None


@custom_op("c2d::conv2d_igemm", mutates_args=("out",), device_types=_CU)
def conv2d_igemm(x: Tensor, weight: Tensor, kpad: int, cout: int, ksize: int, stride: int, up: bool,
                 x2: Optional[Tensor], gn_scale: Optional[Tensor], gn_shift: Optional[Tensor], gn_silu: bool,
                 ln_stats: Optional[Tensor], ln_gamma: Optional[Tensor], ln_beta: Optional[Tensor], silu_in: bool,
                 bias: Optional[Tensor], act: int, temb: Optional[Tensor], resid: Optional[Tensor],
                 out: Tensor, src_pad: bool = False, lnf_eps: float = 0.0, gn_mom: Optional[Tensor] = None,
                 gn_groups: int = 0, up_fold: bool = False, pad_after: bool = False) -> None:
    d = _conv_desc(x, weight, kpad, cout, ksize, stride, up, x2, gn_scale, gn_shift, gn_silu, ln_stats, ln_gamma,
                   ln_beta, silu_in, bias, act, temb, resid, out, src_pad, lnf_eps, gn_mom, gn_groups, up_fold,
                   pad_after)
    wsb = lib().c2d_conv2d_igemm_workspace_size(ctypes.byref(d))
    if wsb:
        ws = torch.empty(wsb // 4, device=x.device, dtype=torch.float32)
        d.ws = ptr(ws); d.ws_bytes = wsb
    if _plan_probe is not None:
        tid, ks = ctypes.c_int(), ctypes.c_int()
        check(lib().c2d_conv2d_igemm_plan(ctypes.byref(d), ctypes.byref(tid), ctypes.byref(ks)), "c2d_conv2d_igemm_plan")
        _plan_probe.append((tid.value, ks.value))
    check(lib().c2d_conv2d_igemm(ctypes.byref(d), stream_ptr()), "c2d_conv2d_igemm")


@conv2d_igemm.register_fake
def _(x, weight, kpad, cout, ksize, stride, up, x2, gn_scale, gn_shift, gn_silu, ln_stats, ln_gamma, ln_beta,
      silu_in, bias, act, temb, resid, out, src_pad=False, lnf_eps=0.0, gn_mom=None, gn_groups=0, up_fold=False,
      pad_after=False):
    return None


@custom_op("c2d::pack_weights", mutates_args=("out",), device_types=_CU)
def pack_weights(w: Tensor, cout: int, cin: int, ksize: int, cin_pad: int, kpad: int, out: Tensor) -> None:
    check(lib().c2d_pack_weights(ptr(w), cout, cin, ksize, cin_pad, kpad, ptr(out), stream_ptr()), "c2d_pack_weights")


@custom_op("c2d::groupnorm_stats", mutates_args=("scale", "shift"), device_types=_CU)
def groupnorm_stats(x: Tensor, x2: Optional[Tensor], groups: int, eps: float, gamma: Tensor, beta: Tensor,
                    scale: Tensor, shift: Tensor) -> None:
    n, c0 = x.shape[0], x.shape[-1]
    c1 = x2.shape[-1] if x2 is not None else 0
    hw = x.numel() // (n * c0)
    ws = torch.empty(lib().c2d_groupnorm_workspace_size(n, c0 + c1, hw) // 4, device=x.device, dtype=torch.float32)
    check(lib().c2d_groupnorm_stats(ptr(x), ptr(x2), c0, c1, n, hw, groups, eps, ptr(gamma), ptr(beta), ptr(scale),
                                    ptr(shift), ptr(ws), stream_ptr()), "c2d_groupnorm_stats")


@custom_op("c2d::groupnorm_apply", mutates_args=("out",), device_types=_CU)
def groupnorm_apply(x: Tensor, x2: Optional[Tensor], scale: Tensor, shift: Tensor, silu: bool, out: Tensor) -> None:
    n, c0 = x.shape[0], x.shape[-1]
    c1 = x2.shape[-1] if x2 is not None else 0
    hw = x.numel() // (n * c0)
    check(lib().c2d_groupnorm_apply(ptr(x), ptr(x2), c0, c1, n, hw, ptr(scale), ptr(shift), int(silu), ptr(out),
                                    stream_ptr()), "c2d_groupnorm_apply")


@custom_op("c2d::groupnorm", mutates_args=("out",), device_types=_CU)
def groupnorm(x: Tensor, x2: Optional[Tensor], groups: int, eps: float, gamma: Tensor, beta: Tensor, silu: bool,
              out: Tensor) -> None:
    n, c0 = x.shape[0], x.shape[-1]
    c1 = x2.shape[-1] if x2 is not None else 0
    hw = x.numel() // (n * c0)
    wsb = lib().c2d_groupnorm_run_workspace_size(n, c0 + c1, hw, groups)
    ws = torch.empty((wsb + 15) // 16 * 4, device=x.device, dtype=torch.float32) if wsb else None
    check(lib().c2d_groupnorm(ptr(x), ptr(x2), c0, c1, n, hw, groups, eps, ptr(gamma), ptr(beta), int(silu), ptr(out),
                              ptr(ws), wsb, stream_ptr()), "c2d_groupnorm")


@custom_op("c2d::groupnorm_pad", mutates_args=("out",), device_types=_CU)
def groupnorm_pad(x: Tensor, x2: Optional[Tensor], groups: int, eps: float, gamma: Tensor, beta: Tensor, silu: bool,
                  out: Tensor) -> None:
    n, h, w, c0 = x.shape
    c1 = x2.shape[-1] if x2 is not None else 0
    wsb = lib().c2d_groupnorm_pad_workspace_size(n, c0 + c1, h, w)
    ws = torch.empty((wsb + 15) // 16 * 4, device=x.device, dtype=torch.float32)
    check(lib().c2d_groupnorm_pad(ptr(x), ptr(x2), c0, c1, n, h, w, groups, eps, ptr(gamma), ptr(beta), int(silu),
                                  ptr(out), ptr(ws), wsb, stream_ptr()), "c2d_groupnorm_pad")


@custom_op("c2d::groupnorm_moments", mutates_args=("out",), device_types=_CU)
def groupnorm_moments(x: Tensor, groups: int, eps: float, gamma: Tensor, beta: Tensor, silu: bool, mom: Tensor,
                      rows: int, pad: bool, out: Tensor) -> None:
    n, h, w, c = x.shape
    check(lib().c2d_groupnorm_moments(ptr(x), c, n, h * w, groups, eps, ptr(gamma), ptr(beta), int(silu), ptr(mom),
                                      rows, w + 2 if pad else 0, ptr(out), stream_ptr()), "c2d_groupnorm_moments")


@custom_op("c2d::layernorm_stats", mutates_args=("stats",), device_types=_CU)
def layernorm_stats(x: Tensor, eps: float, stats: Tensor) -> None:
    m, c = x.shape
    check(lib().c2d_layernorm_stats(ptr(x), m, c, x.stride(0), eps, ptr(stats), stream_ptr()), "c2d_layernorm_stats")


@custom_op("c2d::layernorm", mutates_args=("out",), device_types=_CU)
def layernorm(x: Tensor, gamma: Tensor, beta: Tensor, eps: float, out: Tensor) -> None:
    m, c = x.shape
    check(lib().c2d_layernorm(ptr(x), m, c, x.stride(0), eps, ptr(gamma), ptr(beta), ptr(out), out.stride(0),
                              stream_ptr()), "c2d_layernorm")


@custom_op("c2d::attention_fwd", mutates_args=("out",), device_types=_CU)
def attention_fwd(q: Tensor, k: Tensor, v: Tensor, batch: int, heads: int, lq: int, lk: int, d: int, scale: float,
                  key_bias: Optional[Tensor], bias_ld_batch: int, bias_ld_head: int, out: Tensor,
                  bias_ld_query: int = 0) -> None:
    if key_bias is None:
        check(lib().c2d_attention_fwd(ptr(q), q.stride(0), ptr(k), k.stride(0), ptr(v), v.stride(0), ptr(out),
                                      out.stride(0), batch, heads, lq, lk, d, scale, 1, stream_ptr()), "c2d_attention_fwd")
    else:
        check(lib().c2d_attention_fwd_mask(ptr(q), q.stride(0), ptr(k), k.stride(0), ptr(v), v.stride(0), ptr(out),
                                           out.stride(0), batch, heads, lq, lk, d, scale, 1, ptr(key_bias),
                                           bias_ld_batch, bias_ld_head, bias_ld_query, stream_ptr()),
              "c2d_attention_fwd_mask")


@custom_op("c2d::attention_small", mutates_args=("out",), device_types=_CU)
def attention_small(q: Tensor, k: Tensor, v: Tensor, batch: int, heads: int, l: int, d: int, scale: float,
                    causal: bool, out: Tensor) -> None:
    check(lib().c2d_attention_small(ptr(q), q.stride(0), ptr(k), k.stride(0), ptr(v), v.stride(0), ptr(out),
                                    out.stride(0), batch, heads, l, d, scale, int(causal), stream_ptr()),
          "c2d_attention_small")


@custom_op("c2d::window_attention", mutates_args=("out",), device_types=_CU)
def window_attention(qkv: Tensor, row_map: Tensor, n_windows: int, heads: int, d: int, bias: Tensor,
                     mask: Optional[Tensor], out: Tensor) -> None:
    n_mask = mask.shape[0] if mask is not None else 0
    check(lib().c2d_window_attention(ptr(qkv), qkv.stride(0), ptr(row_map), n_windows, heads, d, ptr(bias), ptr(mask),
                                     n_mask, ptr(out), out.stride(0), stream_ptr()), "c2d_window_attention")


@custom_op("c2d::htsat_mel_patches", mutates_args=("out",), device_types=_CU)
def htsat_mel_patches(mel: Tensor, bn_scale: Tensor, bn_shift: Tensor, out: Tensor) -> None:
    b, t, _ = mel.shape
    check(lib().c2d_htsat_mel_patches(ptr(mel), b, t, ptr(bn_scale), ptr(bn_shift), ptr(out), stream_ptr()),
          "c2d_htsat_mel_patches")


@custom_op("c2d::patch_merge_gather", mutates_args=("out",), device_types=_CU)
def patch_merge_gather(x: Tensor, b: int, h: int, w: int, c: int, out: Tensor) -> None:
    check(lib().c2d_patch_merge_gather(ptr(x), b, h, w, c, ptr(out), stream_ptr()), "c2d_patch_merge_gather")


@custom_op("c2d::row_mean", mutates_args=("out",), device_types=_CU)
def row_mean(x: Tensor, b: int, rows: int, out: Tensor) -> None:
    check(lib().c2d_row_mean(ptr(x), b, rows, x.shape[1], x.stride(0), ptr(out), stream_ptr()), "c2d_row_mean")


@custom_op("c2d::softmax_rows", mutates_args=("out",), device_types=_CU)
def softmax_rows(x: Tensor, out: Tensor) -> None:
    check(lib().c2d_softmax_rows(ptr(x), x.shape[0], x.shape[1], x.stride(0), ptr(out), out.stride(0), stream_ptr()),
          "c2d_softmax_rows")


@custom_op("c2d::l2_normalize", mutates_args=("x",), device_types=_CU)
def l2_normalize(x: Tensor) -> None:
    m, c = x.shape
    check(lib().c2d_l2_normalize(ptr(x), m, c, stream_ptr()), "c2d_l2_normalize")


@custom_op("c2d::clap_log_mel", mutates_args=("out",), device_types=_CU)
def clap_log_mel(wave: Tensor, offsets: Tensor, lengths: Tensor, max_len: int, n_fft: int, hop: int, window: Tensor,
                 filters: Tensor, filter_range: Tensor, n_mels: int, out: Tensor) -> None:
    check(lib().c2d_clap_log_mel(ptr(wave), ptr(offsets), ptr(lengths), offsets.numel(), max_len, n_fft, hop,
                                 ptr(window), ptr(filters), ptr(filter_range), n_mels, ptr(out), stream_ptr()),
          "c2d_clap_log_mel")


@custom_op("c2d::timestep_embedding", mutates_args=("out",), device_types=_CU)
def timestep_embedding(t_table: Tensor, step_index: Optional[Tensor], n: int, dim: int, out: Tensor) -> None:
    check(lib().c2d_timestep_embedding(ptr(t_table), ptr(step_index), n, dim, ptr(out), stream_ptr()),
          "c2d_timestep_embedding")


@custom_op("c2d::cfg_ddim_step", mutates_args=("x", "step_index"), device_types=_CU)
def cfg_ddim_step(eps: Tensor, x: Tensor, guidance: float, coef: Tensor, step_index: Tensor, advance: bool) -> None:
    b, c, hgt, wid = x.shape
    check(lib().c2d_cfg_ddim_step(ptr(eps), ptr(x), b, c, hgt * wid, guidance, ptr(coef), ptr(step_index), int(advance),
                                  stream_ptr()), "c2d_cfg_ddim_step")


@custom_op("c2d::latent_to_nhwc", mutates_args=("out",), device_types=_CU)
def latent_to_nhwc(x: Tensor, cpad: int, dup: bool, out: Tensor) -> None:
    b, c, hgt, wid = x.shape
    check(lib().c2d_latent_to_nhwc(ptr(x), b, c, hgt * wid, cpad, int(dup), ptr(out), stream_ptr()),
          "c2d_latent_to_nhwc")


@custom_op("c2d::image_to_nhwc", mutates_args=("out",), device_types=_CU)
def image_to_nhwc(img: Tensor, out: Tensor) -> None:
    n, h, w, _ = img.shape
    check(lib().c2d_image_to_nhwc(ptr(img), n, h * w, ptr(out), stream_ptr()), "c2d_image_to_nhwc")


@custom_op("c2d::vae_posterior_noise", mutates_args=("x",), device_types=_CU)
def vae_posterior_noise(moments: Tensor, eps: Optional[Tensor], noise: Optional[Tensor], coef: Optional[Tensor],
                        step_index: Optional[Tensor], scaling: float, x: Tensor) -> None:
    n = x.shape[0]
    hw = x.numel() // (4 * n)
    check(lib().c2d_vae_posterior_noise(ptr(moments), moments.stride(0), ptr(eps), ptr(noise), ptr(coef),
                                        ptr(step_index), n, hw, scaling, ptr(x), stream_ptr()),
          "c2d_vae_posterior_noise")


@custom_op("c2d::cfg_ddim_step_masked", mutates_args=("x", "step_index"), device_types=_CU)
def cfg_ddim_step_masked(eps: Tensor, x: Tensor, z0: Tensor, noise: Tensor, mask: Tensor, guidance: float,
                         coef: Tensor, step_index: Tensor, advance: bool) -> None:
    b, _, hgt, wid = x.shape
    check(lib().c2d_cfg_ddim_step_masked(ptr(eps), ptr(x), ptr(z0), ptr(noise), ptr(mask), b, hgt * wid,
                                         coef.shape[0], guidance, ptr(coef), ptr(step_index), int(advance),
                                         stream_ptr()), "c2d_cfg_ddim_step_masked")


@custom_op("c2d::mask_to_latent", mutates_args=("out",), device_types=_CU)
def mask_to_latent(mask_u8: Tensor, out: Tensor) -> None:
    n, h, w = out.shape
    check(lib().c2d_mask_to_latent(ptr(mask_u8), n, h, w, ptr(out), stream_ptr()), "c2d_mask_to_latent")


@custom_op("c2d::composite_u8", mutates_args=("out",), device_types=_CU)
def composite_u8(decoded: Tensor, original: Tensor, mask_u8: Tensor, out: Tensor) -> None:
    check(lib().c2d_composite_u8(ptr(decoded), ptr(original), ptr(mask_u8), mask_u8.numel(), ptr(out), stream_ptr()),
          "c2d_composite_u8")


@custom_op("c2d::inpaint_prepare", mutates_args=("z0", "x", "mask"), device_types=_CU)
def inpaint_prepare(moments: Tensor, eps: Optional[Tensor], noise: Tensor, mask_u8: Tensor, coef: Optional[Tensor],
                    step_index: Optional[Tensor], pure_noise: bool, scaling: float, z0: Tensor, x: Tensor,
                    mask: Tensor) -> None:
    n, h, w = mask.shape
    check(lib().c2d_inpaint_prepare(ptr(moments), moments.stride(0), ptr(eps), ptr(noise), ptr(mask_u8), ptr(coef),
                                    ptr(step_index), int(pure_noise), n, h, w, scaling, ptr(z0), ptr(x), ptr(mask),
                                    stream_ptr()), "c2d_inpaint_prepare")


@custom_op("c2d::upsample_nearest2x", mutates_args=("out",), device_types=_CU)
def upsample_nearest2x(x: Tensor, out: Tensor) -> None:
    n, h, w, c = x.shape
    check(lib().c2d_upsample_nearest2x(ptr(x), n, h, w, c, ptr(out), stream_ptr()), "c2d_upsample_nearest2x")


@custom_op("c2d::add", mutates_args=("out",), device_types=_CU)
def add(a: Tensor, b: Tensor, out: Tensor) -> None:
    check(lib().c2d_add(ptr(a), ptr(b), ptr(out), a.numel(), stream_ptr()), "c2d_add")


for _op in (pack_weights, groupnorm_stats, groupnorm_apply, groupnorm, groupnorm_pad, groupnorm_moments, layernorm_stats, layernorm, attention_fwd,
            attention_small, window_attention, htsat_mel_patches, patch_merge_gather, row_mean, softmax_rows,
            l2_normalize, clap_log_mel, timestep_embedding, cfg_ddim_step, latent_to_nhwc, upsample_nearest2x, add,
            image_to_nhwc, vae_posterior_noise, cfg_ddim_step_masked, mask_to_latent, composite_u8, inpaint_prepare):
    _op.register_fake(lambda *args, **kwargs: None)

OPS = ("conv2d_igemm", "pack_weights", "groupnorm_stats", "groupnorm_apply", "groupnorm", "groupnorm_pad", "groupnorm_moments",
       "layernorm_stats",
       "layernorm", "attention_fwd", "attention_small", "window_attention", "htsat_mel_patches", "patch_merge_gather",
       "row_mean", "softmax_rows", "l2_normalize", "clap_log_mel", "timestep_embedding", "cfg_ddim_step",
       "latent_to_nhwc", "upsample_nearest2x", "add", "image_to_nhwc", "vae_posterior_noise",
       "cfg_ddim_step_masked", "mask_to_latent", "composite_u8", "inpaint_prepare")
```

clap2diffusion_amd/unet.py:

```python
from __future__ import annotations

import os

import torch
import torch.nn as nn

from . import ops
from .layers import HConv2d, HGroupNorm, HLayerNorm, HLinear, HUpConv2d
from .processor import AttnProcessor, AudioAttnProcessor
from .weights import SD15_UNET

FOLD_FF_OUT = os.environ.get("C2D_FOLD_FF_OUT", "1") != "0"
FOLD_LN = os.environ.get("C2D_LN_FOLD", "1") != "0"
FOLD_LN640 = os.environ.get("C2D_LN_FOLD640", "1") != "0"
GN_MOMENTS = os.environ.get("C2D_GN_MOMENTS", "1") != "0"
GN_GROUPS = 32
CFG_PREFIX_MIN = int(os.environ.get("C2D_CFG_PREFIX_MIN", "1"))


class Attention(nn.Module):

    def __init__(self, query_dim: int, cross_attention_dim: int | None = None, heads: int = 8,
                 dim_head: int | None = None, out_bias: bool = True):
        super().__init__()
        dim_head = dim_head or query_dim // heads
        inner = heads * dim_head
        ctx = cross_attention_dim or query_dim
        self.heads, self.dim_head = heads, dim_head
        self.scale = dim_head ** -0.5
        self.is_cross_attention = cross_attention_dim is not None
        self.to_q = HLinear(query_dim, inner, bias=False)
        self.to_k = HLinear(ctx, inner, bias=False)
        self.to_v = HLinear(ctx, inner, bias=False)
        self.to_out = nn.ModuleList([HLinear(inner, query_dim, bias=out_bias), nn.Dropout(0.0)])
        self.spatial_norm = None
        self.norm_cross = None
        self.residual_connection = False
        self.rescale_output_factor = 1.0
        self.upcast_attention = False
        self.upcast_softmax = False
        self.kpad_q = self.to_q.kpad
        self.kpad_kv = self.to_k.kpad
        self.register_buffer("w_qkv", None if self.is_cross_attention else
                             torch.zeros(3 * inner, self.kpad_q, dtype=torch.float16), persistent=False)
        self.register_buffer("w_kv", torch.zeros(2 * inner, self.kpad_kv, dtype=torch.float16), persistent=False)
        self.processor = AttnProcessor()

    @torch.no_grad()
    def finalize(self):
        self.w_kv.copy_(torch.cat([self.to_k.weight, self.to_v.weight], 0))
        if self.w_qkv is not None:
            self.w_qkv.copy_(torch.cat([self.to_q.weight, self.to_k.weight, self.to_v.weight], 0))

    def set_processor(self, processor) -> None:
        self.processor = processor

    def forward(self, hidden_states, encoder_hidden_states=None, attention_mask=None, **cross_attention_kwargs):
        return self.processor(self, hidden_states, encoder_hidden_states=encoder_hidden_states,
                              attention_mask=attention_mask, **cross_attention_kwargs)

    def head_to_batch_dim(self, tensor: torch.Tensor, out_dim: int = 3) -> torch.Tensor:
        b, l, dim = tensor.shape
        h = self.heads
        t = tensor.reshape(b, l, h, dim // h).permute(0, 2, 1, 3)
        return t.reshape(b * h, l, dim // h) if out_dim == 3 else t

    def batch_to_head_dim(self, tensor: torch.Tensor) -> torch.Tensor:
        bh, l, d = tensor.shape
        h = self.heads
        return tensor.reshape(bh // h, h, l, d).permute(0, 2, 1, 3).reshape(bh // h, l, d * h)

    def get_attention_scores(self, query, key, attention_mask=None):
        scores = torch.baddbmm(torch.empty(query.shape[0], query.shape[1], key.shape[1], dtype=query.dtype,
                                           device=query.device), query, key.transpose(-1, -2), beta=0,
                               alpha=self.scale)
        if attention_mask is not None:
            scores = scores + attention_mask
        return scores.softmax(dim=-1).to(query.dtype)


class FeedForward(nn.Module):

    def __init__(self, dim: int, mult: int = 4):
        super().__init__()
        inner = dim * mult
        self.net = nn.ModuleList([nn.Module(), nn.Dropout(0.0), HLinear(inner, dim)])
        self.net[0].proj = HLinear(dim, 2 * inner)

    @torch.no_grad()
    def load_geglu(self, w, b):
        wi, bi = ops.geglu_interleave(w.float(), b.float())
        self.net[0].proj.load(wi, bi)


class BasicTransformerBlock(nn.Module):
    def __init__(self, dim: int, heads: int, cross_dim: int):
        super().__init__()
        self.norm1 = HLayerNorm(dim)
        self.attn1 = Attention(dim, None, heads)
        self.norm2 = HLayerNorm(dim)
        self.attn2 = Attention(dim, cross_dim, heads)
        self.norm3 = HLayerNorm(dim)
        self.ff = FeedForward(dim)
        self.lnf = dim in (320, 640)
        self.lnf_folded = False
        for name in ("qkv", "q", "ff"):
            self.register_buffer(f"lnf_{name}_w", None, persistent=False)
            self.register_buffer(f"lnf_{name}_b", None, persistent=False)

    @torch.no_grad()
    def finalize(self) -> None:
        if not (self.lnf and FOLD_LN):
            return
        c = self.norm1.c
        wq = torch.cat([self.attn1.to_q.weight, self.attn1.to_k.weight, self.attn1.to_v.weight], 0)
        for name, w, b, norm in (("qkv", wq, None, self.norm1), ("q", self.attn2.to_q.weight, None, self.norm2),
                                 ("ff", self.ff.net[0].proj.weight, self.ff.net[0].proj.bias, self.norm3)):
            wf, bf = ops.fold_layernorm(w, b, norm.weight, norm.bias, c)
            setattr(self, f"lnf_{name}_w", wf.contiguous())
            setattr(self, f"lnf_{name}_b", bf.contiguous())
        self.lnf_folded = True

    def _lnf_on(self, m: int, cout: int, geglu: bool) -> bool:
        c = self.norm1.c
        if not (self.lnf_folded and ops.panel_gemm(m, c, cout, geglu, lnfold=True)):
            return False
        if ops.panel_gemm(m, c, cout, geglu) or (c == 320 and m >= 8192):
            return True
        if c == 640 and m >= 8192 and FOLD_LN640:
            panels = (m + 127) // 128
            ns = min(max((256 + panels - 1) // panels, 1), ((cout >> 5) + 7) // 8)
            return panels * ns <= 256
        return False

    def _attend(self, attn: Attention, x, h, ehs, mask, kwargs):
        if getattr(attn.processor, "fuses_residual", False):
            return attn(x, encoder_hidden_states=ehs, attention_mask=mask, _residual=h, **kwargs)
        out = attn(x, encoder_hidden_states=ehs, attention_mask=mask, **kwargs)
        return ops.add(out.to(h.dtype).contiguous(), h)

    def forward(self, h: torch.Tensor, ehs: torch.Tensor, cross_attention_kwargs: dict,
                encoder_attention_mask: torch.Tensor | None = None,
                cfg_dup: torch.Tensor | None = None) -> torch.Tensor:
        h = self.forward_attn(h, ehs, cross_attention_kwargs, encoder_attention_mask, cfg_dup)
        b, l, c = h.shape
        h2 = h.view(b * l, c)
        self.ff.net[2](self.ff_inner(h2), resid=h2, out=h2)
        return h

    def ff_inner(self, h2: torch.Tensor) -> torch.Tensor:
        proj = self.ff.net[0].proj
        if self._lnf_on(h2.shape[0], proj.out_features, True):
            return ops.conv(h2, self.lnf_ff_w, proj.kpad, proj.out_features, ksize=1, bias=self.lnf_ff_b,
                            act="geglu", ln_fold=self.norm3.eps)
        return proj(self.norm3(h2), act="geglu")

    def forward_attn(self, h: torch.Tensor, ehs: torch.Tensor, cross_attention_kwargs: dict,
                     encoder_attention_mask: torch.Tensor | None = None,
                     cfg_dup: torch.Tensor | None = None) -> torch.Tensor:
        kw = cross_attention_kwargs or {}
        b, l, c = h.shape
        inner = self.attn1.heads * self.attn1.dim_head
        if type(self.attn1.processor) is AttnProcessor and self._lnf_on(b * l, 3 * inner, False):
            qkv = ops.conv(h.view(b * l, c), self.lnf_qkv_w, self.attn1.kpad_q, 3 * inner, ksize=1,
                           bias=self.lnf_qkv_b, ln_fold=self.norm1.eps)
            h = self._attend(self.attn1, h, h, None, None, dict(kw, _qkv=qkv))
        else:
            h = self._attend(self.attn1, self.norm1(h), h, None, None, kw)
        if cfg_dup is not None:
            n = h.shape[0]
            if h.data_ptr() != cfg_dup.data_ptr():
                cfg_dup[:n].copy_(h)
            cfg_dup[n:].copy_(cfg_dup[:n])
            h = cfg_dup
        b, l, c = h.shape
        if type(self.attn2.processor) in (AttnProcessor, AudioAttnProcessor) and self._lnf_on(b * l, inner, False):
            q = ops.conv(h.view(b * l, c), self.lnf_q_w, self.attn2.kpad_q, inner, ksize=1, bias=self.lnf_q_b,
                         ln_fold=self.norm2.eps)
            return self._attend(self.attn2, h, h, ehs, encoder_attention_mask, dict(kw, _q=q))
        return self._attend(self.attn2, self.norm2(h), h, ehs, encoder_attention_mask, kw)


class Transformer2DModel(nn.Module):
    def __init__(self, c: int, heads: int, cross_dim: int, groups: int = 32):
        super().__init__()
        self.norm = HGroupNorm(groups, c, 1e-6)
        self.proj_in = HConv2d(c, c, 1)
        self.transformer_blocks = nn.ModuleList([BasicTransformerBlock(c, heads, cross_dim)])
        self.proj_out = HConv2d(c, c, 1)
        self.fold_kpad = ops.kpad_of(5 * c)
        self.fold_ok = c % 64 == 0
        self.register_buffer("w_out_fold", torch.zeros(c, self.fold_kpad, dtype=torch.float16), persistent=False)
        self.register_buffer("b_out_fold", torch.zeros(c, dtype=torch.float32), persistent=False)

    @torch.no_grad()
    def finalize(self) -> None:
        for blk in self.transformer_blocks:
            blk.finalize()
        if not self.fold_ok:
            return
        c = self.proj_out.cout
        wp = self.proj_out.weight[:, :c].float()
        ff2 = self.transformer_blocks[0].ff.net[2]
        w2 = ff2.weight[:, :4 * c].float()
        self.w_out_fold.copy_(torch.cat([wp, wp @ w2], 1).to(torch.float16))
        self.b_out_fold.copy_(wp @ ff2.bias.float() + self.proj_out.bias.float())

    def _block_out(self, t: torch.Tensor, x4: torch.Tensor, resid: torch.Tensor, gm: int = 0):
        blk = self.transformer_blocks[0]
        b, l, c = t.shape
        hh, ww = x4.shape[1], x4.shape[2]
        t2 = t.view(b * l, c)
        ff1 = blk.ff_inner(t2)
        r = ops.conv(t2.view(b, hh, ww, c), self.w_out_fold, self.fold_kpad, c, ksize=1, bias=self.b_out_fold,
                     x2=ff1.view(b, hh, ww, ff1.shape[-1]), resid=resid.reshape(b, hh, ww, c),
                     gn_moments=gm)
        return r

    def forward(self, x, ehs, cross_attention_kwargs, encoder_attention_mask=None,
                cfg_dup: torch.Tensor | None = None, x_mom=None, want_mom: bool = False):
        gm = GN_GROUPS if want_mom and GN_MOMENTS else 0
        r = self._forward(x, ehs, cross_attention_kwargs, encoder_attention_mask, cfg_dup, x_mom, gm)
        if want_mom and not gm:
            return r, None
        return r

    def _forward(self, x, ehs, cross_attention_kwargs, encoder_attention_mask, cfg_dup, x_mom, gm):
        n, hh, ww, c = x.shape
        blk = self.transformer_blocks[0]
        fold = FOLD_FF_OUT and self.fold_ok
        if cfg_dup is None:
            h = self.proj_in(self.norm.apply(x, mom=x_mom))
            if fold:
                t = blk.forward_attn(h.view(n, hh * ww, c), ehs, cross_attention_kwargs, encoder_attention_mask)
                return self._block_out(t, x, x, gm)
            t = blk(h.view(n, hh * ww, c), ehs, cross_attention_kwargs, encoder_attention_mask)
            return self.proj_out(t.view(n, hh, ww, c), resid=x, gn_moments=gm)
        hb = x.new_empty((2 * n, hh * ww, c))
        h = self.proj_in(self.norm.apply(x, mom=x_mom), out=hb[:n].view(n, hh, ww, c))
        if fold:
            t = blk.forward_attn(h.view(n, hh * ww, c), ehs, cross_attention_kwargs, encoder_attention_mask,
                                 cfg_dup=hb)
            cfg_dup[n:].copy_(cfg_dup[:n])
            return self._block_out(t, cfg_dup, cfg_dup, gm)
        t = blk(h.view(n, hh * ww, c), ehs, cross_attention_kwargs, encoder_attention_mask, cfg_dup=hb)
        cfg_dup[n:].copy_(cfg_dup[:n])
        return self.proj_out(t.view(2 * n, hh, ww, c), resid=cfg_dup, gn_moments=gm)


class ResnetBlock2D(nn.Module):
    def __init__(self, cin: int, cout: int, temb_ch: int = 1280, groups: int = 32, eps: float = 1e-5):
        super().__init__()
        self.cin, self.cout = cin, cout
        self.norm1 = HGroupNorm(groups, cin, eps)
        self.conv1 = HConv2d(cin, cout, 3)
        self.time_emb_proj = HLinear(temb_ch, cout) if temb_ch else None
        self.norm2 = HGroupNorm(groups, cout, eps)
        self.dropout = nn.Dropout(0.0)
        self.conv2 = HConv2d(cout, cout, 3)
        self.conv_shortcut = HConv2d(cin, cout, 1) if cin != cout else None
        self.temb_off = None

    def forward(self, x, temb_all=None, skip=None, out=None, x_mom=None, want_mom: bool = False):
        temb = None
        if temb_all is not None:
            temb = temb_all[:, self.temb_off:self.temb_off + self.cout]
        n, hh, ww, _ = x.shape
        cin = self.cin
        p1 = ops.rowring_conv(n, hh, ww, cin, self.cout)
        a1 = self.norm1.apply(x, skip, silu=True, pad=p1, mom=x_mom if skip is None else None)
        if GN_MOMENTS:
            h, hm = self.conv1(a1, temb=temb, padded=p1, gn_moments=self.norm2.num_groups)
        else:
            h, hm = self.conv1(a1, temb=temb, padded=p1), None
        res = self.conv_shortcut(x, x2=skip) if self.conv_shortcut is not None else x
        p2 = ops.rowring_conv(n, hh, ww, self.cout, self.cout)
        y = self.conv2(self.norm2.apply(h, silu=True, pad=p2, mom=hm), resid=res, out=out, padded=p2,
                       gn_moments=self.norm2.num_groups if want_mom and GN_MOMENTS else 0)
        return (y, None) if want_mom and not GN_MOMENTS else y


class Downsample2D(nn.Module):
    def __init__(self, c):
        super().__init__()
        self.conv = HConv2d(c, c, 3, stride=2)

    def forward(self, x, want_mom: bool = False):
        if want_mom and GN_MOMENTS:
            return self.conv(x, gn_moments=GN_GROUPS)
        return (self.conv(x), None) if want_mom else self.conv(x)


class Upsample2D(nn.Module):

    def __init__(self, c):
        super().__init__()
        self.conv = HUpConv2d(c, c)

    def forward(self, x):
        n, h, w, c = x.shape
        if ops.upfold_ok(n, h, w, c, self.conv.cout):
            return self.conv.forward_folded(x)
        return self.conv(ops.upsample_nearest2x(x))


class _Block(nn.Module):
    def __init__(self):
        super().__init__()
        self.resnets = nn.ModuleList()
        self.attentions = nn.ModuleList()


class TimestepEmbedding(nn.Module):
    def __init__(self, cin: int, dim: int):
        super().__init__()
        self.linear_1 = HLinear(cin, dim)
        self.linear_2 = HLinear(dim, dim)

    def forward(self, t_sin):
        return self.linear_2(self.linear_1(t_sin, act="silu"))


class UNetOutput:
    def __init__(self, sample):
        self.sample = sample

    def __getitem__(self, i):
        return (self.sample,)[i]


class UNet2DConditionModel(nn.Module):
    def __init__(self, cfg: dict = SD15_UNET):
        super().__init__()
        self.cfg = dict(cfg)
        ch = cfg["block_out_channels"]
        heads, ctx, groups = cfg["heads"], cfg["cross_attention_dim"], cfg["norm_groups"]
        temb_ch = ch[0] * 4
        self.in_pad = 8
        self.conv_in = HConv2d(cfg["in_channels"], ch[0], 3, cin_pad=self.in_pad)
        self.time_embedding = TimestepEmbedding(ch[0], temb_ch)
        self.down_blocks = nn.ModuleList()
        out_c = ch[0]
        for i, c in enumerate(ch):
            blk = _Block()
            in_c, out_c = out_c, c
            for j in range(cfg["layers_per_block"]):
                blk.resnets.append(ResnetBlock2D(in_c if j == 0 else out_c, out_c, temb_ch, groups))
                if cfg["attn_blocks"][i]:
                    blk.attentions.append(Transformer2DModel(out_c, heads, ctx, groups))
            if i < len(ch) - 1:
                blk.downsamplers = nn.ModuleList([Downsample2D(out_c)])
            self.down_blocks.append(blk)
        self.mid_block = _Block()
        self.mid_block.resnets.append(ResnetBlock2D(ch[-1], ch[-1], temb_ch, groups))
        self.mid_block.attentions.append(Transformer2DModel(ch[-1], heads, ctx, groups))
        self.mid_block.resnets.append(ResnetBlock2D(ch[-1], ch[-1], temb_ch, groups))
        self.up_blocks = nn.ModuleList()
        rev = list(reversed(ch))
        rev_attn = list(reversed(cfg["attn_blocks"]))
        out_c = rev[0]
        n_up = cfg["layers_per_block"] + 1
        for i in range(len(rev)):
            blk = _Block()
            prev_c, out_c = out_c, rev[i]
            in_c = rev[min(i + 1, len(rev) - 1)]
            for j in range(n_up):
                skip = in_c if j == n_up - 1 else out_c
                r_in = prev_c if j == 0 else out_c
                blk.resnets.append(ResnetBlock2D(r_in + skip, out_c, temb_ch, groups))
                blk.resnets[-1].skip_ch = skip
                if rev_attn[i]:
                    blk.attentions.append(Transformer2DModel(out_c, heads, ctx, groups))
            if i < len(rev) - 1:
                blk.upsamplers = nn.ModuleList([Upsample2D(out_c)])
            self.up_blocks.append(blk)
        self.conv_norm_out = HGroupNorm(groups, ch[0], cfg["norm_eps"])
        self.conv_out = HConv2d(ch[0], cfg["out_channels"], 3)
        resnets = [m for m in self.modules() if isinstance(m, ResnetBlock2D)]
        off = 0
        for r in resnets:
            r.temb_off = off
            off += r.cout
        self.temb_total = off
        kp = ops.kpad_of(temb_ch)
        self.register_buffer("w_temb_all", torch.zeros(off, kp, dtype=torch.float16), persistent=False)
        self.register_buffer("b_temb_all", torch.zeros(off, dtype=torch.float32), persistent=False)
        self.temb_kpad = kp

    @torch.no_grad()
    def load_diffusers_state_dict(self, sd: dict) -> None:
        used = set()
        for name, m in self.named_modules():
            if isinstance(m, FeedForward):
                k = name + ".net.0.proj"
                m.load_geglu(sd[k + ".weight"], sd[k + ".bias"])
                used |= {k + ".weight", k + ".bias"}
        for name, m in self.named_modules():
            if isinstance(m, (HLinear, HConv2d, HGroupNorm, HLayerNorm)):
                if name.endswith("net.0.proj"):
                    continue
                wk, bk = name + ".weight", name + ".bias"
                m.load(sd[wk], sd.get(bk))
                used |= {wk, bk}
        missing = [k for k in sd if k not in used]
        if missing:
            raise KeyError(f"unused checkpoint keys: {missing[:5]} ...")
        self.finalize()

    @torch.no_grad()
    def finalize(self) -> None:
        for m in self.modules():
            if isinstance(m, (Attention, Transformer2DModel)):
                m.finalize()
        rs = [m for m in self.modules() if isinstance(m, ResnetBlock2D)]
        self.w_temb_all.copy_(torch.cat([r.time_emb_proj.weight for r in rs], 0))
        self.b_temb_all.copy_(torch.cat([r.time_emb_proj.bias for r in rs], 0))

    @property
    def attn_processors(self) -> dict:
        return {f"{n}.processor": m.processor for n, m in self.named_modules() if isinstance(m, Attention)}

    def set_attn_processor(self, processor) -> None:
        for n, m in self.named_modules():
            if isinstance(m, Attention):
                m.set_processor(processor[f"{n}.processor"] if isinstance(processor, dict) else processor)

    def time_conditioning(self, t_sin: torch.Tensor) -> torch.Tensor:
        temb = self.time_embedding(t_sin)
        return ops.conv(temb, self.w_temb_all, self.temb_kpad, self.temb_total, ksize=1, bias=self.b_temb_all,
                        silu_in=True)

    def cfg_shared_prefix_ok(self) -> bool:
        blk = self.down_blocks[0]
        if not len(blk.attentions):
            return False
        return type(blk.attentions[0].transformer_blocks[0].attn1.processor) is AttnProcessor

    def forward_nhwc(self, x: torch.Tensor, t_sin: torch.Tensor | None, ehs: torch.Tensor,
                     cross_attention_kwargs: dict | None = None,
                     encoder_attention_mask: torch.Tensor | None = None,
                     temb_all: torch.Tensor | None = None, cfg_pair: bool = False) -> torch.Tensor:
        kw = cross_attention_kwargs or {}
        em = encoder_attention_mask
        if temb_all is None:
            temb_all = self.time_conditioning(t_sin)
        shared = cfg_pair and x.shape[0] >= CFG_PREFIX_MIN and self.cfg_shared_prefix_ok()
        if cfg_pair and not shared:
            x = torch.cat([x, x], 0)
        if shared:
            n0 = x.shape[0]
            skip0 = x.new_empty((2 * n0, x.shape[1], x.shape[2], self.conv_in.cout))
            h = self.conv_in(x, out=skip0[:n0])
            skip0[n0:].copy_(skip0[:n0])
            skips = [skip0]
        else:
            h = self.conv_in(x)
            skips = [h]
        hm = None
        for i, blk in enumerate(self.down_blocks):
            for j, r in enumerate(blk.resnets):
                pre = shared and i == 0 and j == 0
                if pre:
                    hb = h.new_empty((2 * h.shape[0], h.shape[1], h.shape[2], r.cout))
                    h, hm = r(h, temb_all, out=hb[:h.shape[0]], x_mom=hm, want_mom=True)
                else:
                    h, hm = r(h, temb_all, x_mom=hm, want_mom=True)
                if len(blk.attentions):
                    h, hm = blk.attentions[j](h, ehs, kw, em, cfg_dup=hb if pre else None, x_mom=hm, want_mom=True)
                elif pre:
                    hb[h.shape[0]:].copy_(h)
                    h, hm = hb, None
                skips.append(h)
            if hasattr(blk, "downsamplers"):
                h, hm = blk.downsamplers[0](h, want_mom=True)
                skips.append(h)
        mb = self.mid_block
        h, hm = mb.resnets[0](h, temb_all, x_mom=hm, want_mom=True)
        h, hm = mb.attentions[0](h, ehs, kw, em, x_mom=hm, want_mom=True)
        h = mb.resnets[1](h, temb_all, x_mom=hm)
        for blk in self.up_blocks:
            for j, r in enumerate(blk.resnets):
                h, hm = r(h, temb_all, skip=skips.pop(), want_mom=True)
                if len(blk.attentions):
                    h, hm = blk.attentions[j](h, ehs, kw, em, x_mom=hm, want_mom=True)
                else:
                    hm = None
            if hasattr(blk, "upsamplers"):
                h, hm = blk.upsamplers[0](h), None
        return self.conv_out(self.conv_norm_out.apply(h, silu=True, mom=hm))

    def forward(self, sample: torch.Tensor, timestep, encoder_hidden_states: torch.Tensor,
                cross_attention_kwargs: dict | None = None, return_dict: bool = True,
                encoder_attention_mask: torch.Tensor | None = None):
        n = sample.shape[0]
        x = ops.latent_to_nhwc(sample.float().contiguous(), self.in_pad, dup=False)
        t = torch.as_tensor(timestep, dtype=torch.float32, device=sample.device).reshape(-1)
        if t.numel() == 1:
            t_sin = ops.timestep_embedding(t.contiguous(), None, n, self.cfg["block_out_channels"][0])
        else:
            t_sin = torch.cat([ops.timestep_embedding(t[i:i + 1].contiguous(), None, 1,
                                                      self.cfg["block_out_channels"][0]) for i in range(n)])
        ehs = encoder_hidden_states.to(torch.float16).contiguous()
        em = None
        if encoder_attention_mask is not None:
            em = ((1.0 - encoder_attention_mask.float()) * -10000.0).unsqueeze(1)
        eps = self.forward_nhwc(x, t_sin, ehs, cross_attention_kwargs, em)
        out = eps.permute(0, 3, 1, 2).contiguous()
        return UNetOutput(out) if return_dict else (out,)
```

include/c2d.h:

```cpp
#ifndef C2D_H
#define C2D_H

#include <stddef.h>
#include <stdint.h>

#ifdef __cplusplus
extern "C" {
#endif

#define C2D_OK 0
#define C2D_E_ARG (-1)
#define C2D_E_SHAPE (-2)
#define C2D_E_ALIGN (-3)
#define C2D_E_HIP (-4)

#define C2D_PRO_NONE 0
#define C2D_PRO_GN 1
#define C2D_PRO_LN 2
#define C2D_PRO_SILU 3
#define C2D_PRO_LNFOLD 4

#define C2D_ACT_NONE 0
#define C2D_ACT_GEGLU 1
#define C2D_ACT_GELU 2
#define C2D_ACT_RELU 3
#define C2D_ACT_SILU 4
#define C2D_ACT_QUICK_GELU 5

#define C2D_PAD_SAME 0
#define C2D_PAD_AFTER 1

typedef struct c2d_conv_desc {
    const void* src0;
    const void* src1;
    int c0, c1;
    int n, h, w;
    int oh, ow;
    int ksize;
    int stride;
    int up;
    const void* weight;
    int cout;
    int kpad;
    int pro;
    int pro_silu;
    const float* pro_a;
    const float* pro_b;
    const float* gamma;
    const float* beta;
    const float* bias;
    int act;
    const void* temb;
    int temb_ld;
    const void* resid;
    int resid_ld;
    void* out;
    int out_ld;
    void* ws;
    size_t ws_bytes;
    int src_pad;
    float pro_eps;
    void* gn_mom;
    int gn_groups;
    int pad_mode;
} c2d_conv_desc;

int c2d_conv2d_igemm(const c2d_conv_desc* d, void* stream);

size_t c2d_conv2d_igemm_workspace_size(const c2d_conv_desc* d);

int c2d_conv2d_igemm_plan(const c2d_conv_desc* d, int* tile_id, int* ksplit);

int c2d_conv2d_gn_rows(const c2d_conv_desc* d);

int c2d_set_plan_override(int tile_id, int ksplit);

int c2d_get_plan_override(int* tile_id, int* ksplit);

size_t c2d_groupnorm_workspace_size(int n, int c, int hw);
int c2d_groupnorm_stats(const void* src0, const void* src1, int c0, int c1, int n, int hw,
                        int groups, float eps, const float* gamma, const float* beta,
                        float* scale, float* shift, void* ws, void* stream);

int c2d_groupnorm_apply(const void* src0, const void* src1, int c0, int c1, int n, int hw,
                        const float* scale, const float* shift, int silu, void* out, void* stream);

size_t c2d_groupnorm_run_workspace_size(int n, int c, int hw, int groups);
int c2d_groupnorm(const void* src0, const void* src1, int c0, int c1, int n, int hw, int groups,
                  float eps, const float* gamma, const float* beta, int silu, void* out,
                  void* ws, size_t ws_bytes, void* stream);

size_t c2d_groupnorm_pad_workspace_size(int n, int c, int h, int w);
int c2d_groupnorm_pad(const void* src0, const void* src1, int c0, int c1, int n, int h, int w, int groups,
                      float eps, const float* gamma, const float* beta, int silu, void* out, void* ws,
                      size_t ws_bytes, void* stream);

int c2d_groupnorm_moments(const void* src, int c, int n, int hw, int groups, float eps, const float* gamma,
                          const float* beta, int silu, const float* mom, int rows, int pw, void* out,
                          void* stream);

int c2d_layernorm_stats(const void* x, int m, int c, int ld, float eps, float* stats, void* stream);
int c2d_layernorm(const void* x, int m, int c, int ld, float eps, const float* gamma,
                  const float* beta, void* out, int out_ld, void* stream);

int c2d_attention_fwd(const void* q, int ldq, const void* k, int ldk, const void* v, int ldv,
                      void* o, int ldo, int batch, int heads, int lq, int lk, int d,
                      float scale, int kv_div, void* stream);

int c2d_attention_fwd_bias(const void* q, int ldq, const void* k, int ldk, const void* v, int ldv,
                           void* o, int ldo, int batch, int heads, int lq, int lk, int d, float scale,
                           int kv_div, const float* key_bias, int bias_ld_batch, int bias_ld_head,
                           void* stream);

int c2d_attention_fwd_mask(const void* q, int ldq, const void* k, int ldk, const void* v, int ldv,
                           void* o, int ldo, int batch, int heads, int lq, int lk, int d, float scale,
                           int kv_div, const float* bias, int bias_ld_batch, int bias_ld_head,
                           int bias_ld_query, void* stream);

int c2d_window_attention(const void* qkv, int ld_qkv, const int* row_map, int n_windows,
                         int heads, int d, const float* bias, const float* mask, int n_mask,
                         void* out, int ldo, void* stream);

int c2d_htsat_mel_patches(const float* mel, int b, int t, const float* bn_scale,
                          const float* bn_shift, void* out, void* stream);

int c2d_patch_merge_gather(const void* x, int b, int h, int w, int c, void* out, void* stream);

int c2d_row_mean(const void* x, int b, int rows, int c, int ld, float* out, void* stream);

int c2d_l2_normalize(float* x, int m, int c, void* stream);

int c2d_attention_small(const void* q, int ldq, const void* k, int ldk, const void* v, int ldv, void* o,
                        int ldo, int batch, int heads, int l, int d, float scale, int causal, void* stream);

int c2d_clap_log_mel(const float* wave, const long long* offsets, const int* lengths, int b, int max_len,
                     int n_fft, int hop, const float* window, const float* mel_filters,
                     const int* filter_range, int n_mels, float* out, void* stream);

int c2d_pack_weights(const float* w, int cout, int cin, int ksize, int cin_pad, int kpad, void* out,
                     void* stream);

int c2d_softmax_rows(const void* x, int rows, int cols, int ld, void* out, int ldo, void* stream);

int c2d_timestep_embedding(const float* t_table, const int* step_index, int n, int dim,
                           void* out, void* stream);

int c2d_cfg_ddim_step(const void* eps, float* x, int b, int c, int hw, float guidance,
                      const float* coef, int* step_index, int advance, void* stream);

int c2d_latent_to_nhwc(const float* x, int n, int c, int hw, int cpad, int dup, void* out,
                       void* stream);

int c2d_image_to_nhwc(const uint8_t* img, int n, int hw, void* out, void* stream);

int c2d_vae_posterior_noise(const void* moments, int ld, const float* eps, const float* noise,
                            const float* coef, const int* step_index, int n, int hw, float scaling, float* x,
                            void* stream);

int c2d_cfg_ddim_step_masked(const void* eps, float* x, const float* z0, const float* noise, const float* mask,
                             int b, int hw, int steps, float guidance, const float* coef, int* step_index,
                             int advance, void* stream);

int c2d_mask_to_latent(const uint8_t* mask_u8, int n, int h, int w, float* out, void* stream);

int c2d_composite_u8(const uint8_t* decoded, const uint8_t* original, const uint8_t* mask_u8, size_t npix,
                     uint8_t* out, void* stream);

int c2d_inpaint_prepare(const void* moments, int ld, const float* eps, const float* noise, const uint8_t* mask_u8,
                        const float* coef, const int* step_index, int pure_noise, int n, int h, int w,
                        float scaling, float* z0, float* x, float* mask, void* stream);

int c2d_upsample_nearest2x(const void* x, int n, int h, int w, int c, void* out, void* stream);

int c2d_add(const void* a, const void* b, void* out, size_t n, void* stream);

int c2d_last_hip_error(void);
const char* c2d_version(void);

#ifdef __cplusplus
}
#endif
#endif
```

Baseline: 9.011 images/sec.

## Reuse GroupNorm moments for concatenated skip inputs in UNet up blocks

Adds kernels that build GroupNorm statistics for a channel-concatenated input (hidden state plus skip) by merging per-block moments already produced by upstream convs, using shifted moments for numerical stability. The UNet now carries moments alongside each skip tensor, and asks the preceding block to emit moments at the group granularity needed by the next concat. This is meant to remove the separate statistics pass over the concatenated tensor in up-block resnets. In exchange it adds a more complex merge step in the apply kernel and extra bookkeeping of moments for the stored skips.

New measurement: 9.000 images/sec. Within noise of the previous version (-0.1%).

```diff
diff --git a/clap2diffusion_amd/_lib.py b/clap2diffusion_amd/_lib.py
--- a/clap2diffusion_amd/_lib.py
+++ b/clap2diffusion_amd/_lib.py
@@ -11,6 +11,7 @@
 
 C2D_PRO_NONE, C2D_PRO_GN, C2D_PRO_LN, C2D_PRO_SILU, C2D_PRO_LNFOLD = 0, 1, 2, 3, 4
 C2D_PAD_SAME, C2D_PAD_AFTER = 0, 1
+C2D_GN_MOM0, C2D_GN_MOM1 = 1, 2
 C2D_ACT = {None: 0, "none": 0, "geglu": 1, "gelu": 2, "relu": 3, "silu": 4, "quick_gelu": 5}
 ERRORS = {-1: "C2D_E_ARG", -2: "C2D_E_SHAPE", -3: "C2D_E_ALIGN", -4: "C2D_E_HIP"}
 
@@ -22,6 +23,8 @@
     "c2d_image_to_nhwc", "c2d_vae_posterior_noise",
     "c2d_cfg_ddim_step_masked", "c2d_mask_to_latent", "c2d_composite_u8",
     "c2d_inpaint_prepare",
+    "c2d_groupnorm_moment_rows", "c2d_groupnorm_moment_stats", "c2d_groupnorm_concat_workspace_size",
+    "c2d_groupnorm_concat_moments", "c2d_groupnorm_concat_map", "c2d_groupnorm_concat_stats_host",
 ]
 
 
@@ -69,6 +72,13 @@
         "c2d_groupnorm_pad": ([vp, vp, i, i, i, i, i, i, f, vp, vp, i, vp, vp, sz, vp], i),
         "c2d_conv2d_gn_rows": ([ctypes.POINTER(ConvDesc)], i),
         "c2d_groupnorm_moments": ([vp, i, i, i, i, f, vp, vp, i, vp, i, i, vp, vp], i),
+        "c2d_groupnorm_moment_rows": ([i, i, i], i),
+        "c2d_groupnorm_moment_stats": ([vp, i, i, i, i, vp, vp], i),
+        "c2d_groupnorm_concat_workspace_size": ([i, i, i, i, i, i], sz),
+        "c2d_groupnorm_concat_moments": ([vp, vp, i, i, i, i, i, f, vp, vp, i, i, vp, i, i, vp, i, i, i, vp, vp, sz,
+                                          vp], i),
+        "c2d_groupnorm_concat_map": ([i, i, i, i, i, vp], i),
+        "c2d_groupnorm_concat_stats_host": ([i, i, i, vp, i, i, i, vp, i, i, i, vp], i),
         "c2d_layernorm_stats": ([vp, i, i, i, f, vp, vp], i),
         "c2d_layernorm": ([vp, i, i, i, f, vp, vp, vp, i, vp], i),
         "c2d_attention_fwd": ([vp, i, vp, i, vp, i, vp, i, i, i, i, i, i, f, i, vp], i),
diff --git a/clap2diffusion_amd/csrc/norm.hip b/clap2diffusion_amd/csrc/norm.hip
--- a/clap2diffusion_amd/csrc/norm.hip
+++ b/clap2diffusion_amd/csrc/norm.hip
@@ -7,7 +7,7 @@
     return (float)((c < c0) ? s0[pix * c0 + c] : s1[pix * c1 + (c - c0)]);
 }
 
-template <int CPT, bool GP = false>
+template <int CPT, bool GP = false, bool MM = false>
 __global__ void __launch_bounds__(256) gn_partial_kernel(const f16* __restrict__ s0, const f16* __restrict__ s1,
                                                          int c0, int c1, int hw, int cpg, int rows_per_block,
                                                          float* __restrict__ ws) {
@@ -118,6 +118,12 @@
         for (int g = t; g < groups; g += 256) {
             float a = 0.f, b = 0.f;
             for (int i = 0; i < cpg; ++i) { a += chs[(g * cpg + i) * 2]; b += chs[(g * cpg + i) * 2 + 1]; }
+            if constexpr (MM) {
+                const double nb = (double)(p_end - p_begin) * cpg, m1 = (double)a / nb;
+                const double m2 = (double)b - (double)a * m1;
+                a = (float)((double)gn_read(s0, s1, c0, c1, img, g * cpg) + m1);
+                b = (float)(m2 > 0.0 ? m2 : 0.0);
+            }
             dst[g * 2] = a;
             dst[g * 2 + 1] = b;
         }
@@ -242,6 +248,81 @@
         for (int i = 0; i < 8; ++i) {
             av[q][i] = scale[(size_t)n * cin + c + i];
             bv[q][i] = shift[(size_t)n * cin + c + i];
+        }
+    }
+    if constexpr (PAD) {
+        const int w = pw - 2, ph = hw / w + 2, npix = ph * pw;
+        const size_t pimg = (size_t)n * npix;
+#pragma unroll 2
+        for (int pp = blockIdx.x * R + r0; pp < npix; pp += gridDim.x * R) {
+            const int py = pp / pw, px = pp - py * pw;
+            const bool inner = py >= 1 && py < ph - 1 && px >= 1 && px < pw - 1;
+            const size_t gp = img + (inner ? (py - 1) * w + (px - 1) : 0);
+#pragma unroll
+            for (int q = 0; q < CPT; ++q) {
+                if (!on[q]) continue;
+                f16x8 o = (f16x8){0, 0, 0, 0, 0, 0, 0, 0};
+                if (inner) {
+                    const f16x8 v = *reinterpret_cast<const f16x8*>(src[q] + gp * ld[q]);
+#pragma unroll
+                    for (int j = 0; j < 8; ++j) {
+                        float y = fmaf((float)v[j], av[q][j], bv[q][j]);
+                        if (silu) y = y * __builtin_amdgcn_rcpf(1.0f + __expf(-y));
+                        o[j] = (f16)y;
+                    }
+                }
+                *reinterpret_cast<f16x8*>(out + (pimg + pp) * cin + cc[q]) = o;
+            }
+        }
+        return;
+    }
+#pragma unroll 4
+    for (int pix = blockIdx.x * R + r0; pix < hw; pix += gridDim.x * R) {
+        const size_t gp = img + pix;
+#pragma unroll
+        for (int q = 0; q < CPT; ++q) {
+            if (!on[q]) continue;
+            const f16x8 v = *reinterpret_cast<const f16x8*>(src[q] + gp * ld[q]);
+            f16x8 o;
+#pragma unroll
+            for (int j = 0; j < 8; ++j) {
+                float y = fmaf((float)v[j], av[q][j], bv[q][j]);
+                if (silu) y = y * __builtin_amdgcn_rcpf(1.0f + __expf(-y));
+                o[j] = (f16)y;
+            }
+            *reinterpret_cast<f16x8*>(out + gp * cin + cc[q]) = o;
+        }
+    }
+}
+
+template <int CPT, bool PAD>
+__device__ __forceinline__ void gn_walk(const f16* __restrict__ s0, const f16* __restrict__ s1, int c0, int c1, int hw,
+                                        int cpg, const float* __restrict__ gamma, const float* __restrict__ beta,
+                                        const float* gmr, int silu, f16* __restrict__ out, int pw) {
+    const int cin = c0 + c1, nch = cin >> 3;
+    const int L = nch < 256 ? nch : 256, R = 256 / L;
+    const int t = threadIdx.x, lane_c = t % L, r0 = t / L;
+    const int n = blockIdx.y;
+    const size_t img = (size_t)n * hw;
+    if (r0 >= R) return;
+    float av[CPT][8], bv[CPT][8];
+    const f16* src[CPT];
+    int ld[CPT], cc[CPT];
+    bool on[CPT];
+#pragma unroll
+    for (int q = 0; q < CPT; ++q) {
+        const int ch = lane_c + q * 256;
+        on[q] = ch < nch;
+        cc[q] = (on[q] ? ch : 0) * 8;
+        const int c = cc[q];
+        src[q] = (c < c0) ? (s0 + c) : (s1 + (c - c0));
+        ld[q] = (c < c0) ? c0 : c1;
+#pragma unroll
+        for (int i = 0; i < 8; ++i) {
+            const int gl = (c + i) / cpg;
+            const float sc = gamma[c + i] * gmr[gl * 2 + 1];
+            av[q][i] = sc;
+            bv[q][i] = beta[c + i] - gmr[gl * 2] * sc;
         }
     }
     if constexpr (PAD) {
@@ -372,70 +453,116 @@
     }
     }
     __syncthreads();
-    if (r0 >= R) return;
-    float av[CPT][8], bv[CPT][8];
-    const f16* src[CPT];
-    int ld[CPT], cc[CPT];
-    bool on[CPT];
-#pragma unroll
-    for (int q = 0; q < CPT; ++q) {
-        const int ch = lane_c + q * 256;
-        on[q] = ch < nch;
-        cc[q] = (on[q] ? ch : 0) * 8;
-        const int c = cc[q];
-        src[q] = (c < c0) ? (s0 + c) : (s1 + (c - c0));
-        ld[q] = (c < c0) ? c0 : c1;
-#pragma unroll
-        for (int i = 0; i < 8; ++i) {
-            const int gl = (c + i) / cpg;
-            const float sc = gamma[c + i] * gmr[gl * 2 + 1];
-            av[q][i] = sc;
-            bv[q][i] = beta[c + i] - gmr[gl * 2] * sc;
-        }
-    }
-    if constexpr (PAD) {
-        const int w = pw - 2, ph = hw / w + 2, npix = ph * pw;
-        const size_t pimg = (size_t)n * npix;
-#pragma unroll 2
-        for (int pp = blockIdx.x * R + r0; pp < npix; pp += gridDim.x * R) {
-            const int py = pp / pw, px = pp - py * pw;
-            const bool inner = py >= 1 && py < ph - 1 && px >= 1 && px < pw - 1;
-            const size_t gp = img + (inner ? (py - 1) * w + (px - 1) : 0);
-#pragma unroll
-            for (int q = 0; q < CPT; ++q) {
-                if (!on[q]) continue;
-                f16x8 o = (f16x8){0, 0, 0, 0, 0, 0, 0, 0};
-                if (inner) {
-                    const f16x8 v = *reinterpret_cast<const f16x8*>(src[q] + gp * ld[q]);
-#pragma unroll
-                    for (int j = 0; j < 8; ++j) {
-                        float y = fmaf((float)v[j], av[q][j], bv[q][j]);
-                        if (silu) y = y * __builtin_amdgcn_rcpf(1.0f + __expf(-y));
-                        o[j] = (f16)y;
+    gn_walk<CPT, PAD>(s0, s1, c0, c1, hw, cpg, gamma, beta, gmr, silu, out, pw);
+}
+
+struct GnCatSpan { int first, count, lo, hi; };
+__host__ __device__ inline GnCatSpan gn_cat_span(int g, int cpg, int c0, int src, int f) {
+    int lo = g * cpg, hi = lo + cpg;
+    if (src == 0) {
+        lo = lo < c0 ? lo : c0;
+        hi = hi < c0 ? hi : c0;
+    } else {
+        lo = (lo > c0 ? lo : c0) - c0;
+        hi = (hi > c0 ? hi : c0) - c0;
+    }
+    return {lo / f, (hi - lo) / f, lo, hi};
+}
+
+struct GnAgg { double n, mean, m2; };
+__host__ __device__ inline GnAgg gn_equal_fold(double sh, double S1, double S2, double Q, double K, double nb) {
+    return {K * nb, sh + S1 / K, Q + nb * (S2 - S1 * S1 / K)};
+}
+__host__ __device__ inline GnAgg gn_merge(const GnAgg& a, const GnAgg& b) {
+    if (a.n == 0.0) return b;
+    if (b.n == 0.0) return a;
+    const double N = a.n + b.n, d = b.mean - a.mean;
+    return {N, a.mean + d * (b.n / N), a.m2 + b.m2 + d * d * (a.n * b.n / N)};
+}
+
+struct GnCatSrc {
+    const float* mom;
+    int groups, nblk, rows;
+};
+
+template <int CPT, bool PAD>
+__global__ void __launch_bounds__(256) gn_apply_cat_kernel(const f16* __restrict__ s0, const f16* __restrict__ s1,
+                                                           int c0, int c1, int hw, int cpg, float eps,
+                                                           const float* __restrict__ gamma,
+                                                           const float* __restrict__ beta, GnCatSrc m0, GnCatSrc m1,
+                                                           int silu, f16* __restrict__ out, int pw) {
+    __shared__ double dacc[256 * 6];
+    __shared__ float gmr[512];
+    const int groups = (c0 + c1) / cpg, parts = 256 / groups;
+    const int t = threadIdx.x, n = blockIdx.y;
+    if (t < parts * groups) {
+        const int g = t % groups, pt = t / groups;
+#pragma unroll
+        for (int src = 0; src < 2; ++src) {
+            const GnCatSrc& m = src ? m1 : m0;
+            double a = 0.0, b = 0.0, qq = 0.0;
+            const int ci = src ? c1 : c0;
+            const GnCatSpan sp = ci > 0 ? gn_cat_span(g, cpg, c0, src, ci / m.groups) : GnCatSpan{0, 0, 0, 0};
+            if (sp.count > 0) {
+                const float2* wp = reinterpret_cast<const float2*>(m.mom) + (size_t)n * m.nblk * m.groups + sp.first;
+                const double sh = (double)wp[0].x;
+                const int dk = parts / sp.count, dj = parts - dk * sp.count;
+                int k = pt / sp.count, j = pt - k * sp.count;
+                while (k < m.nblk) {
+                    float2 v[8];
+                    bool ok[8];
+#pragma unroll
+                    for (int u = 0; u < 8; ++u) {
+                        ok[u] = k < m.nblk;
+                        v[u] = ok[u] ? wp[(size_t)k * m.groups + j] : make_float2(0.f, 0.f);
+                        k += dk;
+                        j += dj;
+                        if (j >= sp.count) { j -= sp.count; ++k; }
+                    }
+#pragma unroll
+                    for (int u = 0; u < 8; ++u) {
+                        if (!ok[u]) continue;
+                        const double d = (double)v[u].x - sh;
+                        a += d;
+                        b += d * d;
+                        qq += (double)v[u].y;
                     }
                 }
-                *reinterpret_cast<f16x8*>(out + (pimg + pp) * cin + cc[q]) = o;
-            }
-        }
-        return;
-    }
-#pragma unroll 4
-    for (int pix = blockIdx.x * R + r0; pix < hw; pix += gridDim.x * R) {
-        const size_t gp = img + pix;
-#pragma unroll
-        for (int q = 0; q < CPT; ++q) {
-            if (!on[q]) continue;
-            const f16x8 v = *reinterpret_cast<const f16x8*>(src[q] + gp * ld[q]);
-            f16x8 o;
-#pragma unroll
-            for (int j = 0; j < 8; ++j) {
-                float y = fmaf((float)v[j], av[q][j], bv[q][j]);
-                if (silu) y = y * __builtin_amdgcn_rcpf(1.0f + __expf(-y));
-                o[j] = (f16)y;
-            }
-            *reinterpret_cast<f16x8*>(out + gp * cin + cc[q]) = o;
-        }
-    }
+            }
+            dacc[t * 6 + src * 3] = a;
+            dacc[t * 6 + src * 3 + 1] = b;
+            dacc[t * 6 + src * 3 + 2] = qq;
+        }
+    }
+    __syncthreads();
+    if (t < groups) {
+        GnAgg agg[2];
+#pragma unroll
+        for (int src = 0; src < 2; ++src) {
+            const GnCatSrc& m = src ? m1 : m0;
+            const int ci = src ? c1 : c0;
+            const GnCatSpan sp = ci > 0 ? gn_cat_span(t, cpg, c0, src, ci / m.groups) : GnCatSpan{0, 0, 0, 0};
+            agg[src] = GnAgg{0.0, 0.0, 0.0};
+            if (sp.count > 0) {
+                double a = 0.0, b = 0.0, qq = 0.0;
+                for (int pt = 0; pt < parts; ++pt) {
+                    const int u = (pt * groups + t) * 6 + src * 3;
+                    a += dacc[u];
+                    b += dacc[u + 1];
+                    qq += dacc[u + 2];
+                }
+                const double sh = (double)m.mom[((size_t)n * m.nblk * m.groups + sp.first) * 2];
+                agg[src] = gn_equal_fold(sh, a, b, qq, (double)m.nblk * sp.count, (double)m.rows * (ci / m.groups));
+            }
+        }
+        const GnAgg all = gn_merge(agg[0], agg[1]);
+        double var = all.m2 / all.n;
+        if (var < 0.0) var = 0.0;
+        gmr[t * 2] = (float)all.mean;
+        gmr[t * 2 + 1] = (float)(1.0 / sqrt(var + (double)eps));
+    }
+    __syncthreads();
+    gn_walk<CPT, PAD>(s0, s1, c0, c1, hw, cpg, gamma, beta, gmr, silu, out, pw);
 }
 
 template <int NT>
@@ -866,6 +993,180 @@
         if (pw) C2D_GNM(2, true); else C2D_GNM(2, false);
     }
 #undef C2D_GNM
+    return check_launch();
+}
+
+static int gn_mom_rows(int n, int c, int hw) {
+    int r = gn_rows_per_block(n, c, hw, tuning().gn_fold_cap);
+    if (r > hw) r = hw;
+    while (hw % r) --r;
+    return r;
+}
+
+static bool gn_mom_stats_shape_ok(int c, int n, int hw, int groups) {
+    return !(c & 7) && c > 0 && (c >> 3) <= 512 && groups > 0 && groups <= 256 && c % groups == 0 && n > 0 && hw > 0;
+}
+
+extern "C" int c2d_groupnorm_moment_rows(int n, int c, int hw) {
+    if (n <= 0 || c <= 0 || (c & 7) || hw <= 0) return 0;
+    return gn_mom_rows(n, c, hw);
+}
+
+static int gn_moment_stats_run(const void* src, int c, int n, int hw, int groups, float* mom, hipStream_t s) {
+    const int nch = c >> 3, cpg = c / groups, rows = gn_mom_rows(n, c, hw);
+    const dim3 grid(hw / rows, n);
+    if (nch <= 256) {
+        const size_t lds = ((size_t)(256 / nch) * c * 2 + (size_t)c * 2) * sizeof(float);
+        hipLaunchKernelGGL((gn_partial_kernel<1, true, true>), grid, dim3(256), lds, s, (const f16*)src,
+                           (const f16*)nullptr, c, 0, hw, cpg, rows, mom);
+    } else {
+        hipLaunchKernelGGL((gn_partial_kernel<2, true, true>), grid, dim3(256), (size_t)c * 2 * sizeof(float), s,
+                           (const f16*)src, (const f16*)nullptr, c, 0, hw, cpg, rows, mom);
+    }
+    return check_launch();
+}
+
+extern "C" int c2d_groupnorm_moment_stats(const void* src, int c, int n, int hw, int groups, float* mom, void* stream) {
+    if (!src || !mom) return C2D_E_ARG;
+    if (!gn_mom_stats_shape_ok(c, n, hw, groups)) return C2D_E_SHAPE;
+    if (!aligned16(src) || ((uintptr_t)mom & 7)) return C2D_E_ALIGN;
+    return gn_moment_stats_run(src, c, n, hw, groups, mom, (hipStream_t)stream);
+}
+
+static int gn_gcd(int a, int b) {
+    while (b) { const int r = a % b; a = b; b = r; }
+    return a;
+}
+
+static int gn_cat_fine(int c0, int c1, int groups) { return gn_gcd((c0 + c1) / groups, c0); }
+
+static bool gn_cat_aligned(int c0, int c1, int groups, int groups0, int groups1) {
+    if (groups0 <= 0 || groups1 <= 0 || c0 % groups0 || c1 % groups1) return false;
+    const int cpg = (c0 + c1) / groups, f0 = c0 / groups0, f1 = c1 / groups1;
+    for (int g = 0; g < groups; ++g) {
+        const GnCatSpan a = gn_cat_span(g, cpg, c0, 0, f0), b = gn_cat_span(g, cpg, c0, 1, f1);
+        if (a.lo % f0 || a.hi % f0 || b.lo % f1 || b.hi % f1) return false;
+    }
+    return true;
+}
+
+static bool gn_cat_shape_ok(int c0, int c1, int n, int hw, int groups) {
+    const int cin = c0 + c1;
+    return !(c0 & 7) && !(c1 & 7) && c0 > 0 && c1 > 0 && (cin >> 3) <= 512 && groups > 0 && groups <= 256 &&
+           cin % groups == 0 && n > 0 && hw > 0;
+}
+
+extern "C" int c2d_groupnorm_concat_map(int c0, int c1, int groups, int groups0, int groups1, int* map) {
+    if (!map) return C2D_E_ARG;
+    if (!gn_cat_shape_ok(c0, c1, 1, 1, groups) || !gn_cat_aligned(c0, c1, groups, groups0, groups1)) return C2D_E_SHAPE;
+    const int cpg = (c0 + c1) / groups;
+    for (int g = 0; g < groups; ++g) {
+        const GnCatSpan a = gn_cat_span(g, cpg, c0, 0, c0 / groups0), b = gn_cat_span(g, cpg, c0, 1, c1 / groups1);
+        map[g * 4] = a.first; map[g * 4 + 1] = a.count; map[g * 4 + 2] = b.first; map[g * 4 + 3] = b.count;
+    }
+    return C2D_OK;
+}
+
+extern "C" int c2d_groupnorm_concat_stats_host(int c0, int c1, int groups, const float* mom0, int groups0, int nblk0,
+                                               int rows0, const float* mom1, int groups1, int nblk1, int rows1,
+                                               double* mean_var) {
+    if (!mom0 || !mom1 || !mean_var) return C2D_E_ARG;
+    if (!gn_cat_shape_ok(c0, c1, 1, 1, groups) || !gn_cat_aligned(c0, c1, groups, groups0, groups1)) return C2D_E_SHAPE;
+    if (nblk0 <= 0 || nblk1 <= 0 || rows0 <= 0 || rows1 <= 0) return C2D_E_SHAPE;
+    const int cpg = (c0 + c1) / groups;
+    for (int g = 0; g < groups; ++g) {
+        GnAgg agg[2] = {{0.0, 0.0, 0.0}, {0.0, 0.0, 0.0}};
+        for (int src = 0; src < 2; ++src) {
+            const float* mom = src ? mom1 : mom0;
+            const int gs = src ? groups1 : groups0, nblk = src ? nblk1 : nblk0, rows = src ? rows1 : rows0;
+            const int f = (src ? c1 : c0) / gs;
+            const GnCatSpan sp = gn_cat_span(g, cpg, c0, src, f);
+            if (sp.count == 0) continue;
+            const double sh = (double)mom[(size_t)sp.first * 2];
+            double a = 0.0, b = 0.0, qq = 0.0;
+            for (int k = 0; k < nblk; ++k)
+                for (int j = 0; j < sp.count; ++j) {
+                    const float* e = mom + ((size_t)k * gs + sp.first + j) * 2;
+                    const double d = (double)e[0] - sh;
+                    a += d;
+                    b += d * d;
+                    qq += (double)e[1];
+                }
+            agg[src] = gn_equal_fold(sh, a, b, qq, (double)nblk * sp.count, (double)rows * f);
+        }
+        const GnAgg all = gn_merge(agg[0], agg[1]);
+        mean_var[g * 2] = all.mean;
+        mean_var[g * 2 + 1] = all.m2 / all.n;
+    }
+    return C2D_OK;
+}
+
+static size_t gn_cat_src_ws(int n, int c, int hw, int fine_groups) {
+    const size_t b = (size_t)n * (hw / gn_mom_rows(n, c, hw)) * fine_groups * 2 * sizeof(float);
+    return (b + 15) & ~(size_t)15;
+}
+
+extern "C" size_t c2d_groupnorm_concat_workspace_size(int n, int c0, int c1, int hw, int groups, int flags) {
+    if (!gn_cat_shape_ok(c0, c1, n, hw, groups)) return 0;
+    const int f = gn_cat_fine(c0, c1, groups);
+    size_t b = 0;
+    if (!(flags & C2D_GN_MOM0)) b += gn_cat_src_ws(n, c0, hw, c0 / f);
+    if (!(flags & C2D_GN_MOM1)) b += gn_cat_src_ws(n, c1, hw, c1 / f);
+    return b;
+}
+
+extern "C" int c2d_groupnorm_concat_moments(const void* src0, const void* src1, int c0, int c1, int n, int hw,
+                                            int groups, float eps, const float* gamma, const float* beta, int silu,
+                                            int flags, const float* mom0, int groups0, int rows0, const float* mom1,
+                                            int groups1, int rows1, int pw, void* out, void* ws, size_t ws_bytes,
+                                            void* stream) {
+    if (!src0 || !src1 || !gamma || !beta || !out || (flags & ~(C2D_GN_MOM0 | C2D_GN_MOM1))) return C2D_E_ARG;
+    if (((flags & C2D_GN_MOM0) && !mom0) || ((flags & C2D_GN_MOM1) && !mom1)) return C2D_E_ARG;
+    if (!gn_cat_shape_ok(c0, c1, n, hw, groups)) return C2D_E_SHAPE;
+    if (pw && (pw < 3 || hw % (pw - 2))) return C2D_E_SHAPE;
+    const int fine = gn_cat_fine(c0, c1, groups);
+    hipStream_t s = (hipStream_t)stream;
+    GnCatSrc m[2];
+    for (int i = 0; i < 2; ++i) {
+        const bool has = flags & (i ? C2D_GN_MOM1 : C2D_GN_MOM0);
+        const int ci = i ? c1 : c0, rows = has ? (i ? rows1 : rows0) : gn_mom_rows(n, ci, hw);
+        const int gs = has ? (i ? groups1 : groups0) : ci / fine;
+        if (gs <= 0 || gs > 256 || ci % gs || rows <= 0 || hw % rows) return C2D_E_SHAPE;
+        m[i] = GnCatSrc{has ? (i ? mom1 : mom0) : nullptr, gs, hw / rows, rows};
+    }
+    if (!gn_cat_aligned(c0, c1, groups, m[0].groups, m[1].groups)) return C2D_E_SHAPE;
+    if (!aligned16(src0) || !aligned16(src1) || !aligned16(out)) return C2D_E_ALIGN;
+    if (((uintptr_t)m[0].mom | (uintptr_t)m[1].mom) & 7) return C2D_E_ALIGN;
+    if (!m[0].mom || !m[1].mom) {
+        if (!ws || !aligned16(ws) || ws_bytes < c2d_groupnorm_concat_workspace_size(n, c0, c1, hw, groups, flags))
+            return C2D_E_ARG;
+        char* w = static_cast<char*>(ws);
+        for (int i = 0; i < 2; ++i) {
+            if (m[i].mom) continue;
+            const int ci = i ? c1 : c0;
+            const int rc = gn_moment_stats_run(i ? src1 : src0, ci, n, hw, m[i].groups, reinterpret_cast<float*>(w), s);
+            if (rc != C2D_OK) return rc;
+            m[i].mom = reinterpret_cast<const float*>(w);
+            w += gn_cat_src_ws(n, ci, hw, m[i].groups);
+        }
+    }
+    const int cin = c0 + c1, nch = cin >> 3, cpg = cin / groups;
+    const int L = nch < 256 ? nch : 256, R = 256 / L;
+    const int npix = pw ? (hw / (pw - 2) + 2) * pw : hw;
+    int bx = ((n < 8 ? tuning().gn_fold_apply_blocks : gn_apply_blocks()) + n - 1) / n;
+    const int maxb = (npix + R - 1) / R;
+    if (bx > maxb) bx = maxb;
+    if (bx < 1) bx = 1;
+    const dim3 agrid(bx, n);
+#define C2D_GNC(C, PD)                                                                                             \
+    hipLaunchKernelGGL((gn_apply_cat_kernel<C, PD>), agrid, dim3(256), 0, s, (const f16*)src0, (const f16*)src1, c0, c1, \
+                       hw, cpg, eps, gamma, beta, m[0], m[1], silu, (f16*)out, pw)
+    if (nch <= 256) {
+        if (pw) C2D_GNC(1, true); else C2D_GNC(1, false);
+    } else {
+        if (pw) C2D_GNC(2, true); else C2D_GNC(2, false);
+    }
+#undef C2D_GNC
     return check_launch();
 }
 
diff --git a/clap2diffusion_amd/layers.py b/clap2diffusion_amd/layers.py
--- a/clap2diffusion_amd/layers.py
+++ b/clap2diffusion_amd/layers.py
@@ -92,8 +92,9 @@
         return ops.group_norm_stats(x, self.num_groups, self.eps, self.weight, self.bias, x2=x2)
 
     def apply(self, x: torch.Tensor, x2: torch.Tensor | None = None, silu: bool = False,
-              pad: bool = False, mom=None) -> torch.Tensor:
-        return ops.group_norm(x, self.num_groups, self.eps, self.weight, self.bias, silu, x2=x2, pad=pad, mom=mom)
+              pad: bool = False, mom=None, skip_mom=None) -> torch.Tensor:
+        return ops.group_norm(x, self.num_groups, self.eps, self.weight, self.bias, silu, x2=x2, pad=pad, mom=mom,
+                              mom2=skip_mom)
 
 
 class HLayerNorm(nn.Module):
diff --git a/clap2diffusion_amd/ops.py b/clap2diffusion_amd/ops.py
--- a/clap2diffusion_amd/ops.py
+++ b/clap2diffusion_amd/ops.py
@@ -5,6 +5,7 @@
 import math
 
 import torch
+from torch._subclasses.fake_tensor import FakeTensor
 
 from . import torch_ops
 from ._lib import C2D_ACT
@@ -137,6 +138,8 @@
     if gn_moments and x.dim() == 4 and act is None and not up and not pad_after and out.is_contiguous():
         rows = gn_moment_rows(out.shape[0], oh, ow, x.shape[-1], cout, ksize, stride, bool(padded), resid is not None,
                               temb is not None, gn_moments, x2.shape[-1] if x2 is not None else 0)
+        if rows and not _gn_operands_ok(out, resid, temb):
+            rows = 0
         if rows:
             mom = torch.empty((out.shape[0], oh * ow // rows, gn_moments, 2), device=x.device, dtype=torch.float32)
     C2D.conv2d_igemm(x, weight, kpad, cout, ksize, stride, up, x2, gs, gh, gn_silu, ls, lg, lb, silu_in, bias,
@@ -152,9 +155,22 @@
     def __init__(self, of: torch.Tensor, mom: torch.Tensor, rows: int, groups: int):
         self.of, self.mom, self.rows, self.groups = of, mom, rows, groups
 
+    def covers(self, x: torch.Tensor) -> bool:
+        return x is self.of and x.dim() == 4 and tuple(self.mom.shape[:1]) == tuple(x.shape[:1])
+
     def matches(self, x: torch.Tensor, groups: int) -> bool:
-        return (x is self.of and groups == self.groups and x.dim() == 4 and
-                tuple(self.mom.shape[:1]) == tuple(x.shape[:1]))
+        return self.covers(x) and groups == self.groups
+
+
+def _gn_operands_ok(out: torch.Tensor, resid, temb) -> bool:
+    for t in (out, resid, temb):
+        if t is None:
+            continue
+        if t.stride(-2) % 8:
+            return False
+        if not isinstance(t, FakeTensor) and t.data_ptr() % 16:
+            return False
+    return True
 
 
 @functools.lru_cache(maxsize=None)
@@ -295,11 +311,58 @@
     return out
 
 
+def group_norm_moment_stats(x: torch.Tensor, groups: int, out: torch.Tensor | None = None) -> "GnMoments":
+    _require(x, "x")
+    from ._lib import lib
+    n, h, w, c = x.shape
+    rows = int(lib().c2d_groupnorm_moment_rows(n, c, h * w))
+    if out is None:
+        out = torch.empty((n, h * w // rows, groups, 2), device=x.device, dtype=torch.float32)
+    assert tuple(out.shape) == (n, h * w // rows, groups, 2) and out.is_contiguous()
+    C2D.groupnorm_moment_stats(x, groups, out)
+    return GnMoments(x, out, rows, groups)
+
+
+@functools.lru_cache(maxsize=None)
+def gn_single_launch(n: int, c: int, hw: int, groups: int) -> bool:
+    from ._lib import lib
+    return c % groups == 0 and int(lib().c2d_groupnorm_run_workspace_size(n, c, hw, groups)) == 0
+
+
+@functools.lru_cache(maxsize=None)
+def gn_concat_groups(c0: int, c1: int, groups: int) -> int:
+    return c0 // math.gcd((c0 + c1) // groups, c0 // groups)
+
+
+@functools.lru_cache(maxsize=None)
+def gn_concat_ok(c0: int, c1: int, groups: int, groups0: int, groups1: int) -> bool:
+    import ctypes
+    from ._lib import lib
+    if (c0 + c1) % groups:
+        return False
+    fine = math.gcd((c0 + c1) // groups, c0)
+    buf = (ctypes.c_int * (4 * groups))()
+    return lib().c2d_groupnorm_concat_map(c0, c1, groups, groups0 or c0 // fine, groups1 or c1 // fine, buf) == 0
+
+
 def group_norm(x: torch.Tensor, groups: int, eps: float, gamma: torch.Tensor, beta: torch.Tensor, silu: bool,
                x2: torch.Tensor | None = None, out: torch.Tensor | None = None, pad: bool = False,
-               mom: "GnMoments | None" = None) -> torch.Tensor:
+               mom: "GnMoments | None" = None, mom2: "GnMoments | None" = None) -> torch.Tensor:
     _require(x, "x")
     c = x.shape[-1] + (x2.shape[-1] if x2 is not None else 0)
+    if x2 is not None and x.dim() == 4:
+        m0 = mom if mom is not None and mom.covers(x) else None
+        m1 = mom2 if mom2 is not None and mom2.covers(x2) else None
+        n, h, w, _ = x.shape
+        use = m0 is not None and m1 is not None and (pad or not gn_single_launch(n, c, h * w, groups))
+        if use and gn_concat_ok(x.shape[-1], x2.shape[-1], groups, m0.groups if m0 else 0, m1.groups if m1 else 0):
+            if out is None:
+                out = torch.empty((n, h + 2, w + 2, c) if pad else (n, h, w, c), device=x.device, dtype=F16)
+            C2D.groupnorm_concat_moments(x, x2, groups, float(eps), gamma, beta, bool(silu),
+                                         m0.mom if m0 else None, m0.groups if m0 else 0, m0.rows if m0 else 0,
+                                         m1.mom if m1 else None, m1.groups if m1 else 0, m1.rows if m1 else 0,
+                                         bool(pad), out)
+            return out
     if mom is not None and x2 is None and mom.matches(x, groups):
         n, h, w, _ = x.shape
         if out is None:
diff --git a/clap2diffusion_amd/torch_ops.py b/clap2diffusion_amd/torch_ops.py
--- a/clap2diffusion_amd/torch_ops.py
+++ b/clap2diffusion_amd/torch_ops.py
@@ -5,7 +5,7 @@
 from torch import Tensor
 from torch.library import custom_op
 
-from ._lib import C2D_PAD_AFTER, C2D_PAD_SAME, C2D_PRO_GN, C2D_PRO_LN, C2D_PRO_LNFOLD, C2D_PRO_NONE, C2D_PRO_SILU, ConvDesc, check, lib, ptr, stream_ptr
+from ._lib import C2D_GN_MOM0, C2D_GN_MOM1, C2D_PAD_AFTER, C2D_PAD_SAME, C2D_PRO_GN, C2D_PRO_LN, C2D_PRO_LNFOLD, C2D_PRO_NONE, C2D_PRO_SILU, ConvDesc, check, lib, ptr, stream_ptr
 
 _CU = "cuda"
 
@@ -61,12 +61,12 @@
 _plan_probe: Optional[list] = None
 
 
-@custom_op("c2d::conv2d_igemm", mutates_args=("out",), device_types=_CU)
+@custom_op("c2d::conv2d_igemm", mutates_args=("out", "gn_mom"), device_types=_CU)
 def conv2d_igemm(x: Tensor, weight: Tensor, kpad: int, cout: int, ksize: int, stride: int, up: bool,
                  x2: Optional[Tensor], gn_scale: Optional[Tensor], gn_shift: Optional[Tensor], gn_silu: bool,
                  ln_stats: Optional[Tensor], ln_gamma: Optional[Tensor], ln_beta: Optional[Tensor], silu_in: bool,
                  bias: Optional[Tensor], act: int, temb: Optional[Tensor], resid: Optional[Tensor],
-                 out: Tensor, src_pad: bool = False, lnf_eps: float = 0.0, gn_mom: Optional[Tensor] = None,
+                 out: Tensor, src_pad: bool, lnf_eps: float, gn_mom: Optional[Tensor],
                  gn_groups: int = 0, up_fold: bool = False, pad_after: bool = False) -> None:
     d = _conv_desc(x, weight, kpad, cout, ksize, stride, up, x2, gn_scale, gn_shift, gn_silu, ln_stats, ln_gamma,
                    ln_beta, silu_in, bias, act, temb, resid, out, src_pad, lnf_eps, gn_mom, gn_groups, up_fold,
@@ -84,7 +84,7 @@
 
 @conv2d_igemm.register_fake
 def _(x, weight, kpad, cout, ksize, stride, up, x2, gn_scale, gn_shift, gn_silu, ln_stats, ln_gamma, ln_beta,
-      silu_in, bias, act, temb, resid, out, src_pad=False, lnf_eps=0.0, gn_mom=None, gn_groups=0, up_fold=False,
+      silu_in, bias, act, temb, resid, out, src_pad, lnf_eps, gn_mom, gn_groups=0, up_fold=False,
       pad_after=False):
     return None
 
@@ -143,6 +143,28 @@
     n, h, w, c = x.shape
     check(lib().c2d_groupnorm_moments(ptr(x), c, n, h * w, groups, eps, ptr(gamma), ptr(beta), int(silu), ptr(mom),
                                       rows, w + 2 if pad else 0, ptr(out), stream_ptr()), "c2d_groupnorm_moments")
+
+
+@custom_op("c2d::groupnorm_moment_stats", mutates_args=("mom",), device_types=_CU)
+def groupnorm_moment_stats(x: Tensor, groups: int, mom: Tensor) -> None:
+    n, h, w, c = x.shape
+    check(lib().c2d_groupnorm_moment_stats(ptr(x), c, n, h * w, groups, ptr(mom), stream_ptr()),
+          "c2d_groupnorm_moment_stats")
+
+
+@custom_op("c2d::groupnorm_concat_moments", mutates_args=("out",), device_types=_CU)
+def groupnorm_concat_moments(x: Tensor, x2: Tensor, groups: int, eps: float, gamma: Tensor, beta: Tensor, silu: bool,
+                             mom: Optional[Tensor], mom_groups: int, rows: int, mom2: Optional[Tensor],
+                             mom2_groups: int, rows2: int, pad: bool, out: Tensor) -> None:
+    n, h, w, c0 = x.shape
+    c1 = x2.shape[-1]
+    flags = (C2D_GN_MOM0 if mom is not None else 0) | (C2D_GN_MOM1 if mom2 is not None else 0)
+    wsb = lib().c2d_groupnorm_concat_workspace_size(n, c0, c1, h * w, groups, flags)
+    ws = torch.empty(wsb // 4, device=x.device, dtype=torch.float32) if wsb else None
+    check(lib().c2d_groupnorm_concat_moments(ptr(x), ptr(x2), c0, c1, n, h * w, groups, eps, ptr(gamma), ptr(beta),
+                                             int(silu), flags, ptr(mom), mom_groups, rows, ptr(mom2), mom2_groups,
+                                             rows2, w + 2 if pad else 0, ptr(out), ptr(ws), wsb, stream_ptr()),
+          "c2d_groupnorm_concat_moments")
 
 
 @custom_op("c2d::layernorm_stats", mutates_args=("stats",), device_types=_CU)
@@ -303,14 +325,15 @@
     check(lib().c2d_add(ptr(a), ptr(b), ptr(out), a.numel(), stream_ptr()), "c2d_add")
 
 
-for _op in (pack_weights, groupnorm_stats, groupnorm_apply, groupnorm, groupnorm_pad, groupnorm_moments, layernorm_stats, layernorm, attention_fwd,
+for _op in (pack_weights, groupnorm_stats, groupnorm_apply, groupnorm, groupnorm_pad, groupnorm_moments, groupnorm_moment_stats,
+            groupnorm_concat_moments, layernorm_stats, layernorm, attention_fwd,
             attention_small, window_attention, htsat_mel_patches, patch_merge_gather, row_mean, softmax_rows,
             l2_normalize, clap_log_mel, timestep_embedding, cfg_ddim_step, latent_to_nhwc, upsample_nearest2x, add,
             image_to_nhwc, vae_posterior_noise, cfg_ddim_step_masked, mask_to_latent, composite_u8, inpaint_prepare):
     _op.register_fake(lambda *args, **kwargs: None)
 
 OPS = ("conv2d_igemm", "pack_weights", "groupnorm_stats", "groupnorm_apply", "groupnorm", "groupnorm_pad", "groupnorm_moments",
-       "layernorm_stats",
+       "groupnorm_moment_stats", "groupnorm_concat_moments", "layernorm_stats",
        "layernorm", "attention_fwd", "attention_small", "window_attention", "htsat_mel_patches", "patch_merge_gather",
        "row_mean", "softmax_rows", "l2_normalize", "clap_log_mel", "timestep_embedding", "cfg_ddim_step",
        "latent_to_nhwc", "upsample_nearest2x", "add", "image_to_nhwc", "vae_posterior_noise",
diff --git a/clap2diffusion_amd/unet.py b/clap2diffusion_amd/unet.py
--- a/clap2diffusion_amd/unet.py
+++ b/clap2diffusion_amd/unet.py
@@ -219,7 +219,7 @@
 
     def forward(self, x, ehs, cross_attention_kwargs, encoder_attention_mask=None,
                 cfg_dup: torch.Tensor | None = None, x_mom=None, want_mom: bool = False):
-        gm = GN_GROUPS if want_mom and GN_MOMENTS else 0
+        gm = (GN_GROUPS if want_mom is True else int(want_mom)) if GN_MOMENTS else 0
         r = self._forward(x, ehs, cross_attention_kwargs, encoder_attention_mask, cfg_dup, x_mom, gm)
         if want_mom and not gm:
             return r, None
@@ -261,14 +261,14 @@
         self.conv_shortcut = HConv2d(cin, cout, 1) if cin != cout else None
         self.temb_off = None
 
-    def forward(self, x, temb_all=None, skip=None, out=None, x_mom=None, want_mom: bool = False):
+    def forward(self, x, temb_all=None, skip=None, out=None, x_mom=None, want_mom: bool | int = False, skip_mom=None):
         temb = None
         if temb_all is not None:
             temb = temb_all[:, self.temb_off:self.temb_off + self.cout]
         n, hh, ww, _ = x.shape
         cin = self.cin
         p1 = ops.rowring_conv(n, hh, ww, cin, self.cout)
-        a1 = self.norm1.apply(x, skip, silu=True, pad=p1, mom=x_mom if skip is None else None)
+        a1 = self.norm1.apply(x, skip, silu=True, pad=p1, mom=x_mom, skip_mom=skip_mom)
         if GN_MOMENTS:
             h, hm = self.conv1(a1, temb=temb, padded=p1, gn_moments=self.norm2.num_groups)
         else:
@@ -276,7 +276,7 @@
         res = self.conv_shortcut(x, x2=skip) if self.conv_shortcut is not None else x
         p2 = ops.rowring_conv(n, hh, ww, self.cout, self.cout)
         y = self.conv2(self.norm2.apply(h, silu=True, pad=p2, mom=hm), resid=res, out=out, padded=p2,
-                       gn_moments=self.norm2.num_groups if want_mom and GN_MOMENTS else 0)
+                       gn_moments=(self.norm2.num_groups if want_mom is True else int(want_mom)) if GN_MOMENTS else 0)
         return (y, None) if want_mom and not GN_MOMENTS else y
 
 
@@ -452,11 +452,14 @@
             skip0 = x.new_empty((2 * n0, x.shape[1], x.shape[2], self.conv_in.cout))
             h = self.conv_in(x, out=skip0[:n0])
             skip0[n0:].copy_(skip0[:n0])
-            skips = [skip0]
         else:
-            h = self.conv_in(x)
-            skips = [h]
-        hm = None
+            h = skip0 = self.conv_in(x)
+        hm = sm = None
+        if GN_MOMENTS and not ops.gn_single_launch(h.shape[0], h.shape[-1], h.shape[1] * h.shape[2], GN_GROUPS):
+            hm = sm = ops.group_norm_moment_stats(h, GN_GROUPS)
+            if shared:
+                sm = ops.GnMoments(skip0, hm.mom.repeat(2, 1, 1, 1), hm.rows, GN_GROUPS)
+        skips = [(skip0, sm)]
         for i, blk in enumerate(self.down_blocks):
             for j, r in enumerate(blk.resnets):
                 pre = shared and i == 0 and j == 0
@@ -470,21 +473,31 @@
                 elif pre:
                     hb[h.shape[0]:].copy_(h)
                     h, hm = hb, None
-                skips.append(h)
+                skips.append((h, hm))
             if hasattr(blk, "downsamplers"):
                 h, hm = blk.downsamplers[0](h, want_mom=True)
-                skips.append(h)
+                skips.append((h, hm))
         mb = self.mid_block
         h, hm = mb.resnets[0](h, temb_all, x_mom=hm, want_mom=True)
         h, hm = mb.attentions[0](h, ehs, kw, em, x_mom=hm, want_mom=True)
-        h = mb.resnets[1](h, temb_all, x_mom=hm)
+
+        def cat_groups(r, x):
+            if not GN_MOMENTS or ops.gn_single_launch(x.shape[0], r.cin, x.shape[1] * x.shape[2], r.norm1.num_groups):
+                return 0
+            return ops.gn_concat_groups(r.cin - r.skip_ch, r.skip_ch, r.norm1.num_groups)
+
+        g = cat_groups(self.up_blocks[0].resnets[0], h)
+        h, hm = mb.resnets[1](h, temb_all, x_mom=hm, want_mom=g) if g else (mb.resnets[1](h, temb_all, x_mom=hm), None)
         for blk in self.up_blocks:
+            last = len(blk.resnets) - 1
             for j, r in enumerate(blk.resnets):
-                h, hm = r(h, temb_all, skip=skips.pop(), want_mom=True)
+                skip, sm = skips.pop()
+                nxt = (cat_groups(blk.resnets[j + 1], h) if j < last else 0) or True
                 if len(blk.attentions):
-                    h, hm = blk.attentions[j](h, ehs, kw, em, x_mom=hm, want_mom=True)
+                    h, hm = r(h, temb_all, skip=skip, x_mom=hm, skip_mom=sm, want_mom=True)
+                    h, hm = blk.attentions[j](h, ehs, kw, em, x_mom=hm, want_mom=nxt)
                 else:
-                    hm = None
+                    h, hm = r(h, temb_all, skip=skip, x_mom=hm, skip_mom=sm, want_mom=nxt)
             if hasattr(blk, "upsamplers"):
                 h, hm = blk.upsamplers[0](h), None
         return self.conv_out(self.conv_norm_out.apply(h, silu=True, mom=hm))
diff --git a/include/c2d.h b/include/c2d.h
--- a/include/c2d.h
+++ b/include/c2d.h
@@ -99,6 +99,19 @@
                           const float* beta, int silu, const float* mom, int rows, int pw, void* out,
                           void* stream);
 
+#define C2D_GN_MOM0 1
+#define C2D_GN_MOM1 2
+int c2d_groupnorm_moment_rows(int n, int c, int hw);
+int c2d_groupnorm_moment_stats(const void* src, int c, int n, int hw, int groups, float* mom, void* stream);
+size_t c2d_groupnorm_concat_workspace_size(int n, int c0, int c1, int hw, int groups, int flags);
+int c2d_groupnorm_concat_moments(const void* src0, const void* src1, int c0, int c1, int n, int hw, int groups,
+                                 float eps, const float* gamma, const float* beta, int silu, int flags,
+                                 const float* mom0, int groups0, int rows0, const float* mom1, int groups1,
+                                 int rows1, int pw, void* out, void* ws, size_t ws_bytes, void* stream);
+int c2d_groupnorm_concat_map(int c0, int c1, int groups, int groups0, int groups1, int* map);
+int c2d_groupnorm_concat_stats_host(int c0, int c1, int groups, const float* mom0, int groups0, int nblk0, int rows0,
+                                    const float* mom1, int groups1, int nblk1, int rows1, double* mean_var);
+
 int c2d_layernorm_stats(const void* x, int m, int c, int ld, float eps, float* stats, void* stream);
 int c2d_layernorm(const void* x, int m, int c, int ld, float eps, const float* gamma,
                   const float* beta, void* out, int out_ld, void* stream);
```
